# POSTECH-CVLab/InstaOrder

Measured on AMD Instinct MI355X. Metric: instance-pairs/sec (fwd+bwd), higher is better.
Workload: dtype f32; 1 GPU; InstaOrderNet_o, pair-batch 256 per GPU at 256x256x5, fp32, fwd+bwd+SGD (BASELINE.json configs[1]); inputs=resident in HBM, pairs_per_gpu=256, input_size=256, parallelism=dp1, hip_graph=True, setup_steps=0, inputs_distinct=True

## Files before the change

### include/instaorder_hip.h

```cpp
#ifndef INSTAORDER_HIP_H
#define INSTAORDER_HIP_H

#include <stddef.h>
#include <stdint.h>

#ifdef __cplusplus
extern "C" {
#endif

#define IO_OK 0
#define IO_ERR_SHAPE (-1)
#define IO_ERR_WORKSPACE (-2)
#define IO_ERR_LAUNCH (-3)
#define IO_ERR_STATE (-4)
#define IO_ERR_NODEVICE (-5)

#if !defined(__HIP__) && !defined(HIP_INCLUDE_HIP_HIP_RUNTIME_API_H)
typedef void* hipStream_t;
#endif

int io_abi_version(void);
const char* io_last_error_string(void);
int io_device_count(void);
int io_set_winograd(int on);
// ... 182 lines not shown
int io_depth_errors_median(const float* pred, const uint16_t* gt, int B, int H, int W, float gt_div, float min_depth,
                           float max_depth, double* out, float* medians, void* workspace, size_t workspace_bytes,
                           hipStream_t stream);
int io_disp_sample_points(const float* disp, int B, int H, int W, const int* points, float* values, int* decisions,
                          hipStream_t stream);
#define IO_MASK_NONZERO 0
#define IO_MASK_EQ1 1
#define IO_MASK_MAX_N 65535
int io_mask_pack(const uint8_t* masks, int n, int H, int W, int predicate, int dilate, uint32_t* bits, int64_t* stats,
                 hipStream_t stream);
int io_mask_pair_counts(const uint32_t* p_bits, int n_p, const uint32_t* q_bits, int n_q, int H, int W, int32_t* counts,
                        hipStream_t stream);
#define IO_DEPTH_SELECT_MEAN 0
#define IO_DEPTH_SELECT_MEDIAN 1
size_t io_instance_depth_select_workspace_bytes(int n, int H, int W);
int io_instance_depth_select(const float* disp, int H, int W, const uint8_t* masks, int n, int method, float* value, float* lo,
                             float* hi, int32_t* k, void* workspace, size_t workspace_bytes, hipStream_t stream);
int io_conv2d_fwd_bnstats_dt(const void* x, const void* w, void* y, int N, int H, int W, int Cin, int Cout, int R, int S,
                             int stride, int pad, int G, const float* gamma, const float* beta, float* running_mean,
                             float* running_var, float momentum, float eps, float* mean, float* rstd, float* scale,
                             float* shift, float* workspace, size_t workspace_floats, int dtype, int gw,
                             hipStream_t stream);
int io_conv2d_dgrad_bnbwd_dt(const void* dy, const void* wt, void* dz, int N, int H, int W, int Cin, int Cout, int R, int S,
                             int pad, const void* y, int G, const float* gamma, const float* mean, const float* rstd,
                             const float* scale, const float* shift, float* dgamma, float* dbeta, void* dyb,
                             float* workspace, size_t workspace_floats, int dtype, int gw, hipStream_t stream);
size_t io_stem_packed_floats(int real_channels);
size_t io_stem_wgrad_exact_workspace_bytes(int N, int H, int W, int real_channels);
int io_stem_fwd_bnstats_exact(const float* x8, const float* w, float* y, int N, int H, int W, int real_channels, int G,
                              const float* gamma, const float* beta, float* running_mean, float* running_var,
                              float momentum, float eps, float* mean, float* rstd, float* scale, float* shift,
                              float* workspace, size_t workspace_floats, float* packed, hipStream_t stream);
int io_stem_wgrad_exact(const float* x8, const float* dy, float* dw, int N, int H, int W, int real_channels,
                        void* workspace, size_t workspace_bytes, float* packed, hipStream_t stream);
int io_stem_wgrad_exact_bn(const float* x8, const float* da, const float* y, float* dw, int N, int H, int W,
                           int real_channels, int G, const float* gamma, const float* mean, const float* rstd,
                           const float* scale, const float* shift, float* dgamma, float* dbeta, float* coef,
                           float* bn_partial, size_t bn_partial_floats, void* workspace, size_t workspace_bytes,
                           float* packed, hipStream_t stream);

size_t io_bn_tile_partial_floats(int M, int C, int G);
int io_bn_bwd_coefs_dt(const void* dz, const void* y, int M, int C, int G, const float* gamma, const float* mean,
                       const float* rstd, float* dgamma, float* dbeta, float* coef, float* partial,
                       size_t partial_floats, int dtype, hipStream_t stream);
int io_bn_bwd_coefs_from_tile_partials(float* p1, float* p2, int M, int C, int G, const float* gamma, const float* mean,
                                       const float* rstd, float* dgamma, float* dbeta, float* coef, hipStream_t stream);
typedef struct io_dgrad_fused {
    const void* xb_y;
    const float* xb_coef;
    void* xb_dy_out;
    const void* add;
    const void* relu_mask;
    const void* ep_y;
    const float *ep_mean, *ep_rstd, *ep_scale, *ep_shift;
    void* ep_act_out;
    float *ep_p1, *ep_p2;
    float* wino_scratch;
    size_t wino_scratch_floats;
    const uint32_t* relu_maskbits;
} io_dgrad_fused;
int io_conv2d_dgrad_fused_dt(const void* dy, const void* wt, void* dx, int N, int H, int W, int Cin, int Cout, int R,
                             int S, int pad, int G, const io_dgrad_fused* f, int dtype, hipStream_t stream);
size_t io_conv2d_wino_scratch_floats(int Cin, int Cout);
int io_conv2d_fwd_wino(const float* x, const float* w, float* y, int N, int H, int W, int Cin, int Cout, int G,
                       const float* in_mean, const float* in_scale, const float* in_shift, const float* gamma,
                       const float* beta, float* running_mean, float* running_var, float momentum, float eps, float* mean,
                       float* rstd, float* scale, float* shift, float* workspace, size_t workspace_floats,
                       float* wino_scratch, size_t wino_floats, hipStream_t stream);
int io_conv2d_fwd_xf_dt(const void* x, const void* w, void* y, int N, int H, int W, int Cin, int Cout, int R, int S,
                        int stride, int pad, int G, const float* in_mean, const float* in_scale, const float* in_shift,
                        const float* gamma, const float* beta, float* running_mean, float* running_var, float momentum, float eps,
                        float* mean, float* rstd, float* scale, float* shift, float* workspace, size_t workspace_floats,
                        int dtype, hipStream_t stream);
int io_conv2d_fwd_resid(const float* y3, const float* identity, const float* w, float* y, float* out, int N, int H, int W,
                        int Cin, int Cout, int G, const float* in_mean, const float* in_scale, const float* in_shift,
                        const float* gamma, const float* beta, float* running_mean, float* running_var, float momentum,
                        float eps, float* mean, float* rstd, float* scale, float* shift, float* workspace,
                        size_t workspace_floats, hipStream_t stream);
int io_conv2d_fwd_resid_dt(const void* y3, const void* second, const void* w, void* y, void* out, uint32_t* out_bits, int N,
                           int H, int W, int Cin, int Cout, int G, int two, const float* ta, const float* tb, const float* tc,
                           float* tile_mean, float* tile_m2, int dtype, hipStream_t stream);
int io_set_bf16_p256_xop(int on);
int io_get_bf16_p256_xop(void);
typedef struct io_weight_desc {
    long src, dst_op, dst_t, dst_g;
    int Co, Ci, T, Cop, Cip;
} io_weight_desc;
int io_weights_prepare(const void* table, int n, const float* params, void* ops, int dtype, hipStream_t stream);
int io_weights_unpack_grads(const void* table, int n, const float* gk, float* grads, hipStream_t stream);
size_t io_stem_wgrad_bf16_workspace_bytes(void);
int io_stem_wgrad_bn_bf16(const void* x8, const void* da, const void* y, float* dw, int N, int H, int W, int G,
                          const float* gamma, const float* mean, const float* rstd, const float* scale, const float* shift,
                          float* dgamma, float* dbeta, float* coef, float* bn_partial, size_t bn_partial_floats,
                          void* workspace, size_t workspace_bytes, hipStream_t stream);
int io_debug_last_wgrad_route(void);
int io_maxpool_fwd_xf_dt(const void* x, int N, int H, int W, int C, void* out, uint32_t* idx, int G,
                         const float* in_mean, const float* in_scale, const float* in_shift, int dtype,
                         hipStream_t stream);
int io_conv2d_fwd_bias_dt(const void* x, const void* w, void* y, int N, int H, int W, int Cin, int Cout, int R, int S,
                          int stride, int pad, const float* bias, const void* add, int relu, int dtype, int gw,
                          hipStream_t stream);
int io_maxpool_fwd_dt(const void* x, int N, int H, int W, int C, void* out, uint32_t* idx, int dtype, hipStream_t stream);
int io_maxpool_bwd_dt(const void* dy, const uint32_t* idx, int N, int H, int W, int C, void* dx, int dtype,
                      hipStream_t stream);
int io_avgpool_fc_fwd_dt(const void* x, int N, int HW, int C, const float* w0, const float* b0, int K0, const float* w1,
                         const float* b1, int K1, float* pooled, float* logits, int dtype, hipStream_t stream);
int io_avgpool_fc_bwd_dt(const float* dlogits, const float* pooled, int N, int HW, int C, const float* w0, int K0,
                         const float* w1, int K1, const void* relu_mask, void* dx, float* dw0, float* db0, float* dw1,
                         float* db1, int dtype, hipStream_t stream);

typedef struct io_pair_desc {
    int64_t image_off;
    int64_t mask1_off, mask2_off;
    int32_t H, W;
    int32_t x, y, w, h;
    int32_t flip;
    int32_t interp;
} io_pair_desc;
int io_pair_planes_u8(const uint8_t* arena, size_t arena_bytes, const io_pair_desc* desc_dev,
                      const io_pair_desc* desc_host, int P, int S, const double* mean3, const double* std3, float* rgb,
                      float* modal1, float* modal2, hipStream_t stream);
int io_pair_planes_u8_hw(const uint8_t* arena, size_t arena_bytes, const io_pair_desc* desc_dev,
                         const io_pair_desc* desc_host, int P, int SH, int SW, const double* mean3, const double* std3,
                         float* rgb, float* modal1, float* modal2, hipStream_t stream);

#define IO_RLE_LDS_RUNS 4096
typedef struct io_rle_desc {
    int64_t ends_off;
    int32_t n_runs;
    int32_t H, W;
    int32_t value;
    int64_t out_off;
} io_rle_desc;
int io_rle_decode_u8(const uint32_t* ends_dev, size_t ends_count, const io_rle_desc* desc_dev,
                     const io_rle_desc* desc_host, int n, uint8_t* out, size_t out_bytes, hipStream_t stream);
int io_rle_lds_runs(void);

typedef struct io_prof_entry {
    char name[48];
    long launches;
    double total_ms;
    double flops;
    double bytes;
    double flops_executed;
} io_prof_entry;
int io_prof_begin(void);
int io_prof_begin_ex(int share_events);
int io_prof_end(io_prof_entry* out, int max_entries);
int io_prof_launches(io_prof_entry* out, int max_entries);

#ifdef __cplusplus
}
#endif
#endif
```

### instaorder_amd/_lib.py

```python
import ctypes as C
import os

_HERE = os.path.dirname(os.path.abspath(__file__))
LIB_PATH = os.environ.get("IO_LIB_PATH") or os.path.join(_HERE, "libinstaorder_hip.so")
_lib = None

c_float_p = C.c_void_p


def csrc_digest():
    import glob
    import hashlib
    h = hashlib.sha256()
    files = sorted(glob.glob(os.path.join(_HERE, "csrc", "*.hip")) + glob.glob(os.path.join(_HERE, "csrc", "*.h")))
    files.append(os.path.join(os.path.dirname(_HERE), "include", "instaorder_hip.h"))
    for f in files:
        h.update(os.path.basename(f).encode())
        h.update(open(f, "rb").read())
    return h.hexdigest()[:16]


class TensorInfo(C.Structure):
    _fields_ = [("name", C.c_char * 64), ("kind", C.c_int), ("ndim", C.c_int), ("shape", C.c_long * 4),
                ("offset", C.c_long), ("numel_storage", C.c_long), ("cin_storage", C.c_int),
                ("bn_index", C.c_int), ("running_offset", C.c_long)]


class PairDesc(C.Structure):
    _fields_ = [("image_off", C.c_int64), ("mask1_off", C.c_int64), ("mask2_off", C.c_int64), ("H", C.c_int32),
                ("W", C.c_int32), ("x", C.c_int32), ("y", C.c_int32), ("w", C.c_int32), ("h", C.c_int32),
                ("flip", C.c_int32), ("interp", C.c_int32)]


class RleDesc(C.Structure):
    _fields_ = [("ends_off", C.c_int64), ("n_runs", C.c_int32), ("H", C.c_int32), ("W", C.c_int32),
                ("value", C.c_int32), ("out_off", C.c_int64)]


class DgradFused(C.Structure):
    _fields_ = [(n, C.c_void_p) for n in ("xb_y", "xb_coef", "xb_dy_out", "add", "relu_mask", "ep_y", "ep_mean", "ep_rstd",
                                          "ep_scale", "ep_shift", "ep_act_out", "ep_p1", "ep_p2", "wino_scratch")] + \
               [("wino_scratch_floats", C.c_size_t), ("relu_maskbits", C.c_void_p)]


class ProfEntry(C.Structure):
    _fields_ = [("name", C.c_char * 48), ("launches", C.c_long), ("total_ms", C.c_double),
                ("flops", C.c_double), ("bytes", C.c_double), ("flops_executed", C.c_double)]


class ClipState(C.Structure):
    _fields_ = [("norm", C.c_float), ("coef", C.c_float), ("nonfinite", C.c_int), ("reserved0", C.c_int),
                ("steps", C.c_uint64), ("clipped", C.c_uint64), ("skipped", C.c_uint64), ("reserved", C.c_uint64 * 3)]


_P, _I, _L, _F, _Z = C.c_void_p, C.c_int, C.c_long, C.c_float, C.c_size_t
_D = C.c_double

SIGNATURES = {
    "io_abi_version": (_I, []),
    "io_last_error_string": (C.c_char_p, []),
    "io_device_count": (_I, []),
    "io_set_winograd": (_I, [_I]),
    "io_get_winograd": (_I, []),
    "io_set_bf16_p256": (_I, [_I]),
    "io_get_bf16_p256": (_I, []),
    "io_set_bf16_p256_xop": (_I, [_I]),
    "io_get_bf16_p256_xop": (_I, []),
    "io_conv2d_fwd_resid_dt": (_I, [_P, _P, _P, _P, _P, _P, _I, _I, _I, _I, _I, _I, _I, _P, _P, _P, _P, _P, _I, _P]),
    "io_debug_last_nt_route": (_I, []),
    "io_conv2d_fwd": (_I, [_P, _P, _P, _I, _I, _I, _I, _I, _I, _I, _I, _I, _P]),
    "io_conv2d_bnstats_workspace_floats": (_Z, [_I, _I, _I, _I, _I, _I, _I, _I, _I]),
    "io_conv2d_fwd_bnstats": (_I, [_P, _P, _P, _I, _I, _I, _I, _I, _I, _I, _I, _I, _I, _P, _P, _P, _P, _F, _F, _P, _P,
                                   _P, _P, _P, _Z, _P]),
    "io_conv2d_dgrad": (_I, [_P, _P, _P, _P, _P, _I, _I, _I, _I, _I, _I, _I, _I, _I, _P]),
    "io_conv2d_dgrad_bnbwd": (_I, [_P, _P, _P, _I, _I, _I, _I, _I, _I, _I, _I, _P, _I, _P, _P, _P, _P, _P, _P, _P, _P,
                                   _P, _Z, _P]),
    "io_conv2d_wgrad_workspace_bytes": (_Z, [_I, _I, _I, _I, _I, _I, _I, _I, _I]),
    "io_conv2d_wgrad": (_I, [_P, _P, _P, _I, _I, _I, _I, _I, _I, _I, _I, _I, _P, _Z, _P]),
    "io_filter_transpose": (_I, [_P, _I, _I, _I, _P, _P]),
    "io_bn_partial_floats": (_Z, [_I, _I, _I]),
    "io_bn_stats_finalize": (_I, [_P, _I, _I, _I, _P, _P, _P, _P, _F, _F, _P, _P, _P, _P, _P, _Z, _P]),
    "io_bn_eval_prepare": (_I, [_I, _P, _P, _P, _P, _F, _P, _P, _P, _P]),
    "io_bn_apply": (_I, [_P, _I, _I, _I, _I, _P, _P, _P, _P, _P, _P, _P, _I, _P, _P]),
    "io_bn_bwd": (_I, [_P, _P, _P, _P, _P, _I, _I, _I, _P, _P, _P, _P, _P, _P, _P, _P, _Z, _P, _P]),
    "io_maxpool_fwd": (_I, [_P, _I, _I, _I, _I, _P, _P, _P]),
    "io_maxpool_bwd": (_I, [_P, _P, _I, _I, _I, _I, _P, _P]),
    "io_avgpool_fc_fwd": (_I, [_P, _I, _I, _I, _P, _P, _I, _P, _P, _I, _P, _P, _P]),
    "io_avgpool_fc_bwd": (_I, [_P, _P, _I, _I, _I, _P, _I, _P, _I, _P, _P, _P, _P, _P, _P, _P]),
    "io_pack_planes_nhwc8": (_I, [C.POINTER(C.c_void_p), C.POINTER(C.c_long), _I, _I, _I, _I, _P, _P]),
    "io_pair_planes_u8": (_I, [_P, _Z, _P, _P, _I, _I, _P, _P, _P, _P, _P, _P]),
    "io_pair_planes_u8_hw": (_I, [_P, _Z, _P, _P, _I, _I, _I, _P, _P, _P, _P, _P, _P]),
    "io_rle_decode_u8": (_I, [_P, _Z, _P, _P, _I, _P, _Z, _P]),
    "io_rle_lds_runs": (_I, []),
    "io_order_loss": (_I, [_P, _I, _I, _I, _I, _P, _P, _P, _F, _F, _F, _P, _P, _P]),
    "io_sgd_momentum": (_I, [_P, _P, _P, _Z, _F, _F, _F, _P]),
    "io_adam_step": (_I, [_P, _P, _P, _P, _Z, _D, _D, _D, _F, _F, _D, _D, _P]),
    "io_grad_norm": (_I, [_P, _Z, C.POINTER(C.c_size_t), _I, _F, _P, _Z, _P, _P, _P]),
    "io_grad_norm_workspace_bytes": (_Z, [_Z, _I]),
    "io_grad_norm_chunk_floats": (_I, []),
    "io_sgd_momentum_clipped": (_I, [_P, _P, _P, _Z, _F, _F, _F, _P, _P]),
    "io_adam_step_clipped": (_I, [_P, _P, _P, _P, _Z, _D, _D, _D, _F, _F, _D, _D, _P, _P]),
    "io_net_create": (_P, [_I, _I, C.POINTER(C.c_int)]),
    "io_net_destroy": (None, [_P]),
    "io_net_param_floats": (_L, [_P]),
    "io_net_running_floats": (_L, [_P]),
    "io_net_num_tensors": (_I, [_P]),
    "io_net_tensor_info": (_I, [_P, _I, C.POINTER(TensorInfo)]),
    "io_net_num_logits": (_I, [_P]),
    "io_net_workspace_bytes": (_Z, [_P, _I, _I, _I]),
    "io_net_workspace_bytes_hw": (_Z, [_P, _I, _I, _I]),
    "io_net_forward_eval_hw": (_I, [_P, _P, _P, _P, _I, _I, _I, _P, _Z, _P, _P]),
    "io_net_activation_offset": (_L, [_P, _I, _I, _I]),
    "io_net_forward": (_I, [_P, _P, _P, _P, _I, _I, _I, _I, _P, _Z, _P, _P]),
    "io_net_backward": (_I, [_P, _P, _P, _P, _P, _I, _I, _I, _P, _Z, _P]),
    "io_net_backward_num_stages": (_I, [_P]),
    "io_net_backward_stages": (_I, [_P, _P, _P, _P, _P, _I, _I, _I, _P, _Z, _I, _I, _P]),
    "io_net_set_dtype": (_I, [_P, _I]),
    "io_net_get_dtype": (_I, [_P]),
    "io_pack_planes_nhwc8_dt": (_I, [_P, _P, _I, _I, _I, _I, _P, _I, _P]),
    "io_conv2d_fwd_dt": (_I, [_P, _P, _P, _I, _I, _I, _I, _I, _I, _I, _I, _I, _I, _I, _P]),
    "io_conv2d_dgrad_dt": (_I, [_P, _P, _P, _P, _P, _I, _I, _I, _I, _I, _I, _I, _I, _I, _I, _P]),
    "io_conv2d_wgrad_dt": (_I, [_P, _P, _P, _I, _I, _I, _I, _I, _I, _I, _I, _I, _P, _Z, _I, _I, _P]),
    "io_filter_prepare": (_I, [_P, _I, _I, _I, _P, _I, _I, _P]),
    "io_bn_stats_finalize_dt": (_I, [_P, _I, _I, _I, _P, _P, _P, _P, _F, _F, _P, _P, _P, _P, _P, _Z, _I, _P]),
    "io_bn_apply_dt": (_I, [_P, _I, _I, _I, _I, _P, _P, _P, _P, _P, _P, _P, _I, _P, _I, _P]),
    "io_bn_apply_bits_dt": (_I, [_P, _I, _I, _I, _I, _P, _P, _P, _P, _P, _P, _P, _P, _P, _I, _P]),
    "io_bn_bwd_dt": (_I, [_P, _P, _P, _P, _P, _I, _I, _I, _P, _P, _P, _P, _P, _P, _P, _P, _Z, _P, _I, _P]),
    "io_gconv_pack": (_I, [_P, _I, _I, _I, _P, _P, _I, _P]),
    "io_gconv_unpack_grad": (_I, [_P, _I, _I, _I, _P, _P]),
    "io_gconv2d_fwd": (_I, [_P, _P, _P, _I, _I, _I, _I, _I, _I, _I, _I, _I, _P]),
    "io_gconv2d_dgrad": (_I, [_P, _P, _P, _I, _I, _I, _I, _I, _I, _I, _I, _I, _P]),
    "io_gconv2d_wgrad_workspace_bytes": (_Z, [_I, _I, _I, _I, _I, _I, _I, _I]),
    "io_gconv2d_wgrad": (_I, [_P, _P, _P, _I, _I, _I, _I, _I, _I, _I, _I, _P, _Z, _I, _P]),
    "io_upsample2x_bilinear_fwd": (_I, [_P, _I, _I, _I, _I, _I, _P, _I, _P]),
    "io_upsample2x_bilinear_bwd": (_I, [_P, _I, _I, _I, _I, _I, _P, _I, _P]),
    "io_bias_act": (_I, [_P, _P, _I, _I, _I, _P, _I, _P]),
    "io_relu_bwd": (_I, [_P, _P, _Z, _P, _I, _P]),
    "io_add": (_I, [_P, _P, _Z, _P, _I, _P]),
    "io_colsum_partial_floats": (_Z, [_I, _I]),
    "io_colsum": (_I, [_P, _I, _I, _P, _P, _Z, _I, _P]),
    "io_head1_fwd": (_I, [_P, _I, _I, _I, _P, _P, _I, _P, _I, _P]),
    "io_head1_bwd": (_I, [_P, _P, _P, _I, _I, _I, _P, _I, _P, _P, _P, _P, _Z, _I, _P]),
    "io_conv2d_fwd_bnstats_dt": (_I, [_P, _P, _P, _I, _I, _I, _I, _I, _I, _I, _I, _I, _I, _P, _P, _P, _P, _F, _F, _P,
                                      _P, _P, _P, _P, _Z, _I, _I, _P]),
    "io_conv2d_fwd_bias_dt": (_I, [_P, _P, _P, _I, _I, _I, _I, _I, _I, _I, _I, _I, _P, _P, _I, _I, _I, _P]),
    "io_stem_packed_floats": (_Z, [_I]),
    "io_stem_wgrad_exact_workspace_bytes": (_Z, [_I, _I, _I, _I]),
    "io_stem_fwd_bnstats_exact": (_I, [_P, _P, _P, _I, _I, _I, _I, _I, _P, _P, _P, _P, _F, _F, _P, _P, _P, _P, _P, _Z, _P,
                                       _P]),
# ... 80 lines not shown
```

### instaorder_amd/csrc/capi.hip

```cpp
#include <stdarg.h>
#include <stdio.h>
#include <stdlib.h>
#include <string.h>

#include "io_common.h"

static thread_local char g_err[512] = "";

void io_set_error(const char* fmt, ...) {
    va_list ap;
    va_start(ap, fmt);
    vsnprintf(g_err, sizeof(g_err), fmt, ap);
    va_end(ap);
}

int io_check_launch(const char* what) {
    hipError_t e = hipGetLastError();
    if (e != hipSuccess) {
        io_set_error("%s: %s", what, hipGetErrorString(e));
        return IO_ERR_LAUNCH;
    }
    return IO_OK;
}

extern "C" int io_abi_version(void) { return 1; }

static std::atomic<int> g_wino{-1};
bool io_wino_on() {
    int v = g_wino.load(std::memory_order_relaxed);
    if (v < 0) {
        const char* e = getenv("IO_WINOGRAD");
        v = (e && e[0] == '0') ? 0 : 1;
        g_wino.store(v, std::memory_order_relaxed);
    }
    return v != 0;
}
extern "C" int io_get_winograd(void) { return io_wino_on() ? 1 : 0; }
extern "C" int io_set_winograd(int on) {
    const int prev = io_wino_on() ? 1 : 0;
    g_wino.store(on ? 1 : 0, std::memory_order_relaxed);
    return prev;
}
extern "C" const char* io_last_error_string(void) { return g_err; }

extern "C" int io_device_count(void) {
    int n = 0;
    if (hipGetDeviceCount(&n) != hipSuccess) {
        (void)hipGetLastError();
        return 0;
    }
    int ok = 0;
    for (int i = 0; i < n; ++i) {
        hipDeviceProp_t p;
        if (hipGetDeviceProperties(&p, i) == hipSuccess && strncmp(p.gcnArchName, "gfx950", 6) == 0) ++ok;
    }
    return ok;
}

IoConvGeom io_geom_fwd(int N, int H, int W, int Cin, int Cout, int R, int S, int stride, int pad) {
    IoConvGeom g;
    memset(&g, 0, sizeof(g));
    g.N = N; g.Hi = H; g.Wi = W; g.Ci = Cin;
    g.Ho = (H + 2 * pad - R) / stride + 1;
    g.Wo = (W + 2 * pad - S) / stride + 1;
    g.Co = Cout;
    g.outH = g.Ho; g.outW = g.Wo;
    g.os = 1; g.ooh = 0; g.oow = 0;
    g.is = stride;
    g.Th = R; g.Tw = S;
    g.dh0 = -pad; g.dhs = 1; g.dw0 = -pad; g.dws = 1;
    g.r0 = 0; g.rs = 1; g.s0 = 0; g.ss = 1;
    g.S = S; g.wT = R * S;
    io_geom_finish(g);
    return g;
}

IoConvGeom io_geom_dgrad(int N, int H, int W, int Cin, int Cout, int R, int S, int stride, int pad, int ph,
                         int pw) {
    IoConvGeom g;
    memset(&g, 0, sizeof(g));
    const int Hy = (H + 2 * pad - R) / stride + 1, Wy = (W + 2 * pad - S) / stride + 1;
    g.N = N; g.Hi = Hy; g.Wi = Wy; g.Ci = Cout;
    g.Ho = (H - ph + stride - 1) / stride;
    g.Wo = (W - pw + stride - 1) / stride;
    g.Co = Cin;
    g.outH = H; g.outW = W;
    g.os = stride; g.ooh = ph; g.oow = pw;
    g.is = 1;
    const int rf = (ph + pad) % stride, sf = (pw + pad) % stride;
    g.Th = rf < R ? (R - rf + stride - 1) / stride : 0;
    g.Tw = sf < S ? (S - sf + stride - 1) / stride : 0;
    g.dh0 = (ph + pad - rf) / stride; g.dhs = -1;
    g.dw0 = (pw + pad - sf) / stride; g.dws = -1;
    g.r0 = rf; g.rs = stride; g.s0 = sf; g.ss = stride;
    g.S = S; g.wT = R * S;
    io_geom_finish(g);
    return g;
}

int io_run_dgrad(const void* dy, const void* wt, void* dx, const void* add, const void* mask, int N, int H,
                 int W, int Cin, int Cout, int R, int S, int stride, int pad, hipStream_t st, const IoBwStats* bw,
                 int dt, int gw) {
    IO_REQUIRE(!bw || !bw->y || stride == 1, IO_ERR_SHAPE, "dgrad: fused BN-backward reductions need a stride-1 convolution");
    IO_REQUIRE(!bw || !bw->xb_a || stride == 1 || (R == 1 && S == 1 && pad == 0), IO_ERR_SHAPE,
               "dgrad: the operand transform needs a stride-1 convolution or a strided 1x1 one");
    for (int ph = 0; ph < stride; ++ph)
        for (int pw = 0; pw < stride; ++pw) {
            IoConvGeom g = io_geom_dgrad(N, H, W, Cin, Cout, R, S, stride, pad, ph, pw);
            g.gw = gw;
            if (g.Ho <= 0 || g.Wo <= 0) continue;
            if ((g.Th == 0 || g.Tw == 0) && add == dx && !mask) continue;
            int rc = io_launch_conv_nt(g, dy, wt, dx, add, mask, 0, st, nullptr, nullptr, bw, dt, dt);
            if (rc) return rc;
        }
    return IO_OK;
}

extern "C" int io_conv2d_fwd(const float* x, const float* w, float* y, int N, int H, int W, int Cin, int Cout,
                             int R, int S, int stride, int pad, hipStream_t st) {
    IoConvGeom g = io_geom_fwd(N, H, W, Cin, Cout, R, S, stride, pad);
    return io_launch_conv_nt(g, x, w, y, nullptr, nullptr, Cin == 8, st);
}

// ... 587 lines not shown
```

### instaorder_amd/csrc/conv_igemm.hip

```cpp
#include <string.h>
#include <stdlib.h>

#include "io_common.h"

namespace {

constexpr int kThreads = 256;

__device__ __forceinline__ f32x4 ld4(const float* p) { return *reinterpret_cast<const f32x4*>(p); }
template <typename T> __device__ __forceinline__ void pin(T& v) { asm volatile("" : "+v"(v)); }
__device__ __forceinline__ void st4(float* p, f32x4 v) { *reinterpret_cast<f32x4*>(p) = v; }

__device__ __forceinline__ int xcd_remap(int b, int nwg) {
    const int q = nwg >> 3, r = nwg & 7, x = b & 7, i = b >> 3;
    return (x < r ? x * (q + 1) : r * (q + 1) + (x - r) * q) + i;
}

__device__ __forceinline__ int sdiv(int n, float rd) { return (int)(((float)n + 0.5f) * rd); }
__device__ __forceinline__ int stem_kp(int wT, int cr) { return (wT * cr + 31) / 32 * 32; }
__device__ __forceinline__ int fdiv(int n, IoFastDiv f) {
    return f.shift < 0 ? n : (int)(__umulhi((unsigned)n, f.magic) >> f.shift);
}

typedef unsigned u32x4 __attribute__((ext_vector_type(4)));
constexpr unsigned kInvalidOff = 0xFFFFFFFFu;
constexpr int kStAux = 2;
constexpr int kTrBkm = 64;
constexpr int kTrMinB = 2;
constexpr int kTrStages = 2;
__device__ __forceinline__ __amdgpu_buffer_rsrc_t make_rsrc(const void* p, unsigned bytes) {
    return __builtin_amdgcn_make_buffer_rsrc(const_cast<void*>(p), 0, bytes, 0x00020000);
}
__device__ __forceinline__ __amdgpu_buffer_rsrc_t make_rsrc_at(const void* p, size_t base, size_t total) {
    const size_t rest = total > base ? total - base : 0;
    return make_rsrc(static_cast<const char*>(p) + base, rest > 0xFFFFFFFFull ? 0xFFFFFFFFu : (unsigned)rest);
}
__device__ __forceinline__ f32x4 bld4(__amdgpu_buffer_rsrc_t r, unsigned off) {
    return __builtin_bit_cast(f32x4, __builtin_amdgcn_raw_buffer_load_b128(r, off, 0, 0));
}
template <typename T> __device__ __forceinline__ f32x4 bldv(__amdgpu_buffer_rsrc_t r, unsigned off);
template <> __device__ __forceinline__ f32x4 bldv<float>(__amdgpu_buffer_rsrc_t r, unsigned off) { return bld4(r, off); }
template <> __device__ __forceinline__ f32x4 bldv<bf16_t>(__amdgpu_buffer_rsrc_t r, unsigned off) {
    typedef unsigned u32x2 __attribute__((ext_vector_type(2)));
    const u32x2 q = __builtin_amdgcn_raw_buffer_load_b64(r, off, 0, 0);
    f32x4 v;
    v[0] = __builtin_bit_cast(float, q[0] << 16);
    v[1] = __builtin_bit_cast(float, q[0] & 0xffff0000u);
    v[2] = __builtin_bit_cast(float, q[1] << 16);
    v[3] = __builtin_bit_cast(float, q[1] & 0xffff0000u);
    return v;
}
template <typename T> __device__ __forceinline__ float ld_el(__amdgpu_buffer_rsrc_t r, unsigned off);
template <> __device__ __forceinline__ float ld_el<float>(__amdgpu_buffer_rsrc_t r, unsigned off) {
    return __builtin_bit_cast(float, __builtin_amdgcn_raw_buffer_load_b32(r, off, 0, 0));
}
template <> __device__ __forceinline__ float ld_el<bf16_t>(__amdgpu_buffer_rsrc_t r, unsigned off) {
    return io_bf2f(__builtin_amdgcn_raw_buffer_load_b16(r, off, 0, 0));
}
template <typename T> __device__ __forceinline__ void st_el(float v, __amdgpu_buffer_rsrc_t r, unsigned off);
template <> __device__ __forceinline__ void st_el<float>(float v, __amdgpu_buffer_rsrc_t r, unsigned off) {
    __builtin_amdgcn_raw_buffer_store_b32(__float_as_uint(v), r, off, 0, kStAux);
}
template <> __device__ __forceinline__ void st_el<bf16_t>(float v, __amdgpu_buffer_rsrc_t r, unsigned off) {
    __builtin_amdgcn_raw_buffer_store_b16(io_f2bf(v), r, off, 0, kStAux);
}
template <typename T> __device__ __forceinline__ float ld_el_s(__amdgpu_buffer_rsrc_t r, unsigned off, unsigned soff);
template <> __device__ __forceinline__ float ld_el_s<float>(__amdgpu_buffer_rsrc_t r, unsigned off, unsigned soff) {
    return __builtin_bit_cast(float, __builtin_amdgcn_raw_buffer_load_b32(r, off, soff, 0));
}
template <> __device__ __forceinline__ float ld_el_s<bf16_t>(__amdgpu_buffer_rsrc_t r, unsigned off, unsigned soff) {
    return io_bf2f(__builtin_amdgcn_raw_buffer_load_b16(r, off, soff, 0));
}
template <typename T> __device__ __forceinline__ void st_el_s(float v, __amdgpu_buffer_rsrc_t r, unsigned off, unsigned soff);
template <> __device__ __forceinline__ void st_el_s<float>(float v, __amdgpu_buffer_rsrc_t r, unsigned off, unsigned soff) {
    __builtin_amdgcn_raw_buffer_store_b32(__float_as_uint(v), r, off, soff, kStAux);
}
template <> __device__ __forceinline__ void st_el_s<bf16_t>(float v, __amdgpu_buffer_rsrc_t r, unsigned off, unsigned soff) {
    __builtin_amdgcn_raw_buffer_store_b16(io_f2bf(v), r, off, soff, kStAux);
}
typedef __bf16 bf16x8 __attribute__((ext_vector_type(8)));

template <typename TA, typename TO, int BN, int STEM, int NW, int NBUF = 2, int MINB = 1, bool BWE = false,
          bool XF = false, bool LIN = false, int XB = 0, bool WINO = false>
__global__ __launch_bounds__(NW * 64, MINB) void conv_nt_kernel(IoConvGeom g, const TA* __restrict__ in,
                                                         const TA* __restrict__ wgt, TO* __restrict__ out,
                                                         const TO* __restrict__ add,
                                                         const TO* __restrict__ mask, int ntn, size_t in_bytes,
                                                         unsigned w_bytes, size_t out_bytes,
                                                         float* __restrict__ st_mean, float* __restrict__ st_m2,
                                                         IoBwStats bw) {
    constexpr int ES = sizeof(TA), OS = sizeof(TO);
    constexpr int VE = 16 / ES;
    constexpr bool SWZ = BN == 64;
    constexpr int BM = 128, BK = 128 / ES, LDT = SWZ ? 32 : 32 + 4, NT = NW * 64;
    constexpr int CPT = ES / 2;
    constexpr int TPT = 8 / CPT;
    constexpr bool XK = STEM == 2;
    static_assert(!XK || ES == 4, "the exact-K stem is an fp32 path");
    constexpr int WN = NW / 2;
    static_assert(!WINO || (ES == 4 && OS == 4 && BN == 64 && NW == 4 && STEM == 0 && NBUF == 1 && !LIN && XB == 0),
                  "WINO: fp32, 64-wide tiles, single LDS buffer, plain / XF / BWE forms");
    constexpr int TI = WINO ? 4 : 2, TJ = BN / (32 * WN);
    constexpr int ETI = 2;
    constexpr int AROWS = WINO ? 2 * BM : BM, BROWS = WINO ? 4 * BN : BN;
    constexpr int AR = (BM * 8) / NT;
    constexpr int BR = (BN * 8) / NT;
    constexpr int RS = NT / 8;
    static_assert(TJ >= 1 && BR >= 1, "tile too small for this wave count");
    static_assert(NBUF * (BM + BN) * LDT >= NW * 32 * (BN / WN + 4), "operand LDS too small for the row epilogue");
    extern __shared__ __attribute__((aligned(16))) float smem[];
    float* sA = smem;
    float* sB = smem + NBUF * AROWS * LDT;

    const int tid = threadIdx.x, lane = tid & 63, wave = tid >> 6;
    const int wm = wave / WN, wn = wave % WN;
    const int tile = xcd_remap(blockIdx.x, gridDim.x);
    const int mt = tile / ntn;
    const int m0 = mt * BM, n0 = (tile - mt * ntn) * BN;
    const int HoWo = g.Ho * g.Wo;
    const int M = g.N * HoWo;
    const int lr = tid >> 3, kq = tid & 7;
    const int kw = g.gw ? g.gw : g.Ci;
    const int cbase = g.gw ? n0 : 0;
    const int nkc = STEM ? 1 : kw / BK;
    const int kp = XK ? stem_kp(g.wT, g.cr) : 0;
    const int nk = XK ? kp / 32 : STEM ? (g.wT + TPT - 1) / TPT : (WINO ? g.Th : g.Th * g.Tw) * nkc;

    static_assert(!LIN || STEM == 0, "LIN: regular 1x1 convolutions");
    const int n_lo = LIN ? 0 : fdiv(m0, g.fd_howo);
    const __amdgpu_buffer_rsrc_t rs_in =
        make_rsrc_at(in, LIN ? (size_t)m0 * (size_t)(g.Ci * ES) : (size_t)n_lo * (size_t)(g.Hi * g.Wi) * (size_t)(g.Ci * ES),
                     in_bytes);
    const __amdgpu_buffer_rsrc_t rs_w = make_rsrc(wgt, w_bytes);
    unsigned rowv[AR];
    int hi0[AR], wi0[AR];
    bool rvalid[AR];
#pragma unroll
    for (int j = 0; j < AR; ++j) {
        if constexpr (LIN) {
            rvalid[j] = true;
            hi0[j] = wi0[j] = 0;
            rowv[j] = (unsigned)((lr + RS * j) * g.Ci + kq * VE) * (unsigned)ES;
        } else {
            const int m = m0 + lr + RS * j;
            rvalid[j] = m < M;
            const int mm = rvalid[j] ? m : 0;
            const int n = fdiv(mm, g.fd_howo), rem = mm - n * HoWo;
            const int ho = fdiv(rem, g.fd_wo), wo = rem - ho * g.Wo;
            hi0[j] = ho * g.is;
            wi0[j] = wo * g.is;
            rowv[j] = (unsigned)((((n - n_lo) * g.Hi + hi0[j]) * g.Wi + wi0[j]) * g.Ci + (STEM ? 0 : kq * VE)) * (unsigned)ES;
        }
    }
    constexpr int AI = 2, WBR = 8;
    unsigned wrow[AI];
    int whi[AI];
    bool wl[AI], wr[AI];
    unsigned wvb[WBR];
    f32x4 wa[WINO ? AI : 1][4], wb[WINO ? WBR : 1];
    if constexpr (WINO) {
#pragma unroll
        for (int j = 0; j < AI; ++j) {
            const int m = m0 + 2 * (lr + 32 * j);
            const int n = fdiv(m, g.fd_howo), rem = m - n * HoWo;
            const int ho = fdiv(rem, g.fd_wo), wo = rem - ho * g.Wo;
            whi[j] = ho;
            wl[j] = wo > 0;
            wr[j] = wo + 2 < g.Wi;
            wrow[j] = (unsigned)((((n - n_lo) * g.Hi + ho) * g.Wi + wo) * g.Ci + kq * 4) * 4u;
        }
#pragma unroll
        for (int j = 0; j < WBR; ++j)
            wvb[j] = (unsigned)(((j >> 1) * g.Co + n0 + lr + 32 * (j & 1)) * g.Ci + kq * 4) * 4u;
    }
    unsigned wv[BR];
#pragma unroll
    for (int j = 0; j < BR; ++j)
        wv[j] = XK ? (unsigned)((n0 + lr + RS * j) * kp + kq * VE) * (unsigned)ES
                   : (unsigned)((n0 + lr + RS * j) * g.wT * kw + (STEM ? 0 : kq * VE)) * (unsigned)ES;
    const bool nopad = g.Th == 1 && g.Tw == 1 && g.dh0 == 0 && g.dw0 == 0 && g.is == 1 && g.Hi >= g.Ho &&
                       g.Wi >= g.Wo;

    f32x4 ra[AR], rb[BR];
    static_assert(!XF || STEM == 0, "input transform: regular convolutions");
    static_assert(!XB || (STEM == 0 && !XF), "backward operand transform: regular data gradients, not combined with XF");
    static_assert(XB < 2 || !BWE, "the residual forms are forward paths");
    constexpr bool XT = XF || XB;
    constexpr int XC = ES == 4 ? 1 : 2;
    f32x4 xm[XC], xs[XC], xh[XC];
    f32x4 ry[XB ? AR : 1];
    unsigned xok = 0, xaoff = 0;
    bool xside = false;
    const int xgrp = XF ? m0 / bw.in_Mg : XB ? m0 / bw.xb_Mg : 0;
    const float* const xt_s = XF ? bw.in_scale : bw.xb_a;
    const float* const xt_h = XF ? bw.in_shift : bw.xb_c;
    const float* const xt_m = XF ? bw.in_mean : bw.xb_b;
    const __amdgpu_buffer_rsrc_t rs_xs = make_rsrc(XT ? (const void*)(xt_s + (size_t)xgrp * g.Ci) : (const void*)wgt,
                                                   XT ? (unsigned)g.Ci * 4u : 0u);
    const __amdgpu_buffer_rsrc_t rs_xh = make_rsrc(XT ? (const void*)(xt_h + (size_t)xgrp * g.Ci) : (const void*)wgt,
                                                   XT ? (unsigned)g.Ci * 4u : 0u);
    const __amdgpu_buffer_rsrc_t rs_xm = make_rsrc((XT && xt_m) ? (const void*)(xt_m + (size_t)xgrp * g.Ci)
                                                                : (const void*)wgt,
                                                   (XT && xt_m) ? (unsigned)g.Ci * 4u : 0u);
    const size_t xb_base = LIN ? (size_t)m0 * (size_t)(g.Ci * ES) : (size_t)n_lo * (size_t)(g.Hi * g.Wi) * (size_t)(g.Ci * ES);
    const __amdgpu_buffer_rsrc_t rs_y = make_rsrc_at(XB ? bw.xb_y : (const void*)in, xb_base, XB ? in_bytes : xb_base);
    const __amdgpu_buffer_rsrc_t rs_side =
        make_rsrc_at((XB && bw.xb_out) ? bw.xb_out : (void*)out, xb_base, (XB && bw.xb_out && n0 == 0) ? in_bytes : xb_base);
    int th = 0, tw = 0, cc = 0;
    const float rcr = 1.0f / (float)(XK ? g.cr : 1), rS = 1.0f / (float)g.S;
    auto load_tile = [&](int kt) {
        if constexpr (XK) {
            unsigned eoff[4];
            int edh[4], edw[4];
            bool eok[4];
#pragma unroll
            for (int i = 0; i < 4; ++i) {
                const int e = kt * 32 + kq * 4 + i;
                const int tp = sdiv(e, rcr), ch = e - tp * g.cr;
                eok[i] = tp < g.wT;
                const int r = sdiv(tp, rS), s = tp - r * g.S;
                edh[i] = g.dh0 + g.dhs * r;
                edw[i] = g.dw0 + g.dws * s;
                eoff[i] = (unsigned)((edh[i] * g.Wi + edw[i]) * g.Ci + ch) * 4u;
            }
#pragma unroll
            for (int j = 0; j < AR; ++j)
#pragma unroll
                for (int i = 0; i < 4; ++i) {
                    const int hi = hi0[j] + edh[i], wi = wi0[j] + edw[i];
                    const bool ok = eok[i] && rvalid[j] && (unsigned)hi < (unsigned)g.Hi && (unsigned)wi < (unsigned)g.Wi;
                    ra[j][i] = ld_el<float>(rs_in, ok ? rowv[j] + eoff[i] : kInvalidOff);
                }
#pragma unroll
            for (int j = 0; j < BR; ++j) rb[j] = bld4(rs_w, wv[j] + (unsigned)kt * 128u);
            return;
        }
        if constexpr (LIN) {
            const unsigned koff = (unsigned)(cc * BK) * (unsigned)ES;
            if constexpr (XB) {
                xaoff = koff;
#pragma unroll
                for (int j = 0; j < AR; ++j)
                    ry[j] = __builtin_bit_cast(f32x4, __builtin_amdgcn_raw_buffer_load_b128(rs_y, rowv[j], koff, 0));
            }
            if constexpr (XT) {
                const unsigned coff = (unsigned)(cc * BK + kq * VE) * 4u;
#pragma unroll
                for (int q = 0; q < XC; ++q) {
                    xm[q] = bld4(rs_xm, coff + 16u * q);
                    xs[q] = bld4(rs_xs, coff + 16u * q);
                    xh[q] = bld4(rs_xh, coff + 16u * q);
                }
                xok = ~0u;
            }
#pragma unroll
            for (int j = 0; j < AR; ++j)
                ra[j] = __builtin_bit_cast(f32x4, __builtin_amdgcn_raw_buffer_load_b128(rs_in, rowv[j], koff, 0));
#pragma unroll
            for (int j = 0; j < BR; ++j)
                rb[j] = __builtin_bit_cast(f32x4, __builtin_amdgcn_raw_buffer_load_b128(rs_w, wv[j], koff, 0));
            return;
        }
        if constexpr (WINO) {
            const int dh = g.dh0 + g.dhs * th;
            const unsigned aoff = (unsigned)(((dh * g.Wi - 1) * g.Ci + cc * BK) * 4);
            const unsigned woff = (unsigned)((th * 4 * g.Co * g.Ci + cc * BK) * 4);
            if constexpr (XF) {
                const unsigned coff = (unsigned)(cc * BK + kq * VE) * 4u;
                xm[0] = bld4(rs_xm, coff);
                xs[0] = bld4(rs_xs, coff);
                xh[0] = bld4(rs_xh, coff);
            }
            xok = 0;
#pragma unroll
            for (int j = 0; j < AI; ++j) {
                const bool rowok = (unsigned)(whi[j] + dh) < (unsigned)g.Hi;
#pragma unroll
                for (int i = 0; i < 4; ++i) {
                    const bool ok = rowok & (i == 0 ? wl[j] : i == 3 ? wr[j] : true);
                    xok |= ok ? (1u << (j * 4 + i)) : 0u;
                    wa[j][i] = bld4(rs_in, ok ? wrow[j] + aoff + (unsigned)(i * g.Ci * 4) : kInvalidOff);
                }
            }
#pragma unroll
            for (int j = 0; j < WBR; ++j) wb[j] = bld4(rs_w, wvb[j] + woff);
            return;
        }
        int dh, dw;
        unsigned aoff, woff;
        bool tapok = true;
// ... 72 lines not shown
                    }
                }
                const f32x4 d0 = wa[j][0], d1 = wa[j][1], d2 = wa[j][2], d3 = wa[j][3];
                wa[j][0] = d0 - d2;
                wa[j][1] = d1 + d2;
                wa[j][2] = d2 - d1;
                wa[j][3] = d1 - d3;
            }
            return;
        }
        if constexpr (XF) {
#pragma unroll
            for (int j = 0; j < AR; ++j) {
                const bool ok = (xok >> j) & 1u;
                if constexpr (ES == 4) {
#pragma unroll
                    for (int e = 0; e < 4; ++e) {
                        const float v = fmaxf(__builtin_fmaf(ra[j][e] - xm[0][e], xs[0][e], xh[0][e]), 0.f);
                        ra[j][e] = ok ? v : 0.f;
                    }
                } else {
                    const u32x4 raw = __builtin_bit_cast(u32x4, ra[j]);
                    u32x4 o;
#pragma unroll
                    for (int d = 0; d < 4; ++d) {
                        const int q = d >> 1, e0 = (d & 1) * 2;
                        const float lo = __builtin_bit_cast(float, raw[d] << 16);
                        const float hi = __builtin_bit_cast(float, raw[d] & 0xffff0000u);
                        const float vl = fmaxf(__builtin_fmaf(lo - xm[q][e0], xs[q][e0], xh[q][e0]), 0.f);
                        const float vh = fmaxf(__builtin_fmaf(hi - xm[q][e0 + 1], xs[q][e0 + 1], xh[q][e0 + 1]), 0.f);
                        o[d] = ok ? io_f2bf2(vl, vh) : 0u;
                    }
                    ra[j] = __builtin_bit_cast(f32x4, o);
                }
            }
        }
        if constexpr (XB != 0) {
#pragma unroll
            for (int j = 0; j < AR; ++j) {
                const bool ok = (xok >> j) & 1u;
                if constexpr (XB == 2 && ES == 4) {
#pragma unroll
                    for (int e = 0; e < 4; ++e) {
                        const float v = __builtin_fmaf(ra[j][e] - xm[0][e], xs[0][e], xh[0][e]) + ry[j][e];
                        ra[j][e] = (ok && v > 0.f) ? v : 0.f;
                    }
                } else if constexpr (ES == 4) {
#pragma unroll
                    for (int e = 0; e < 4; ++e) {
                        const float v = __builtin_fmaf(ra[j][e], xs[0][e], __builtin_fmaf(ry[j][e], xm[0][e], xh[0][e]));
                        ra[j][e] = (ok && (XB != 3 || v > 0.f)) ? v : 0.f;
                    }
                } else {
                    const u32x4 raw = __builtin_bit_cast(u32x4, ra[j]), rwy = __builtin_bit_cast(u32x4, ry[j]);
                    u32x4 o;
#pragma unroll
                    for (int d = 0; d < 4; ++d) {
                        const int q = d >> 1, e0 = (d & 1) * 2;
                        const float lo = __builtin_bit_cast(float, raw[d] << 16);
                        const float hi = __builtin_bit_cast(float, raw[d] & 0xffff0000u);
                        const float yl = __builtin_bit_cast(float, rwy[d] << 16);
                        const float yh = __builtin_bit_cast(float, rwy[d] & 0xffff0000u);
                        float vl, vh;
                        if constexpr (XB == 2) {
                            vl = __builtin_fmaf(lo - xm[q][e0], xs[q][e0], xh[q][e0]) + yl;
                            vh = __builtin_fmaf(hi - xm[q][e0 + 1], xs[q][e0 + 1], xh[q][e0 + 1]) + yh;
                        } else {
                            vl = __builtin_fmaf(lo, xs[q][e0], __builtin_fmaf(yl, xm[q][e0], xh[q][e0]));
                            vh = __builtin_fmaf(hi, xs[q][e0 + 1], __builtin_fmaf(yh, xm[q][e0 + 1], xh[q][e0 + 1]));
                        }
                        if constexpr (XB >= 2) {
                            vl = vl > 0.f ? vl : 0.f;
                            vh = vh > 0.f ? vh : 0.f;
                        }
                        o[d] = ok ? io_f2bf2(vl, vh) : 0u;
                    }
                    ra[j] = __builtin_bit_cast(f32x4, o);
                }
            }
            if constexpr (LIN) {
#pragma unroll
                for (int j = 0; j < AR; ++j)
                    __builtin_amdgcn_raw_buffer_store_b128(__builtin_bit_cast(u32x4, ra[j]), rs_side, rowv[j], xaoff, 0);
            } else {
#pragma unroll
                for (int j = 0; j < AR; ++j)
                    __builtin_amdgcn_raw_buffer_store_b128(__builtin_bit_cast(u32x4, ra[j]), rs_side,
                                                           (xside && ((xok >> j) & 1u)) ? rowv[j] + xaoff : kInvalidOff, 0, 0);
            }
        }
    };
    auto store_tile = [&](int buf, bool xdone = false) {
        if constexpr (WINO) {
            if (!xdone) xform_tile();
            float* a = sA + lr * LDT + wchunk * 4;
            float* b = sB + lr * LDT + wchunk * 4;
#pragma unroll
            for (int j = 0; j < AI; ++j)
#pragma unroll
                for (int f = 0; f < 4; ++f) st4(a + (f * 64 + 32 * j) * LDT, wa[j][f]);
#pragma unroll
            for (int j = 0; j < WBR; ++j) st4(b + 32 * j * LDT, wb[j]);
            return;
        }
        float* a = sA + buf * BM * LDT + lr * LDT + wchunk * 4;
        float* b = sB + buf * BN * LDT + lr * LDT + wchunk * 4;
        if constexpr (XT) {
            if (!xdone) xform_tile();
        }
#pragma unroll
        for (int j = 0; j < AR; ++j) st4(a + RS * j * LDT, ra[j]);
#pragma unroll
        for (int j = 0; j < BR; ++j) st4(b + RS * j * LDT, rb[j]);
    };

    f32x16 acc[TI][TJ];
#pragma unroll
    for (int i = 0; i < TI; ++i)
#pragma unroll
        for (int j = 0; j < TJ; ++j)
#pragma unroll
            for (int r = 0; r < 16; ++r) acc[i][j][r] = 0.f;

    const int rsw = SWZ ? (lane >> 1) & 7 : 0;
    const int a_off = (wm * (WINO ? 32 : 64) + (lane & 31)) * LDT + (SWZ ? 0 : (lane >> 5) * 4);
    const int b_off = (wn * (BN / WN) + (lane & 31)) * LDT + (SWZ ? 0 : (lane >> 5) * 4);
    constexpr int FB = WINO ? 4 : TJ;
    auto read_frags = [&](int buf, int kk, f32x4 (&a)[TI], f32x4 (&b)[FB]) {
        const int koff = SWZ ? ((((lane >> 5) + kk * 2) ^ rsw) * 4) : kk * 8;
        if constexpr (WINO) {
#pragma unroll
            for (int f = 0; f < 4; ++f) {
                a[f] = ld4(sA + a_off + koff + f * 64 * LDT);
                b[f] = ld4(sB + b_off + koff + f * 64 * LDT);
            }
            return;
        }
        const float* al = sA + buf * BM * LDT + a_off + koff;
        const float* bl = sB + buf * BN * LDT + b_off + koff;
#pragma unroll
        for (int i = 0; i < TI; ++i) a[i] = ld4(al + i * 32 * LDT);
#pragma unroll
        for (int j = 0; j < TJ; ++j) b[j] = ld4(bl + j * 32 * LDT);
    };
    auto mma16 = [&](const f32x4 (&a)[TI], const f32x4 (&b)[FB]) {
        if constexpr (WINO) {
#pragma unroll
            for (int tt = 0; tt < 4; ++tt)
#pragma unroll
                for (int f = 0; f < 4; ++f)
                    acc[f][0] = __builtin_amdgcn_mfma_f32_32x32x2f32(a[f][tt], b[f][tt], acc[f][0], 0, 0, 0);
        } else if constexpr (ES == 4) {
#pragma unroll
            for (int tt = 0; tt < 4; ++tt)
#pragma unroll
                for (int i = 0; i < TI; ++i)
#pragma unroll
                    for (int j = 0; j < TJ; ++j)
                        acc[i][j] = __builtin_amdgcn_mfma_f32_32x32x2f32(a[i][tt], b[j][tt], acc[i][j], 0, 0, 0);
        } else {
#pragma unroll
            for (int i = 0; i < TI; ++i)
#pragma unroll
                for (int j = 0; j < TJ; ++j)
                    acc[i][j] = __builtin_amdgcn_mfma_f32_32x32x16_bf16(__builtin_bit_cast(bf16x8, a[i]),
                                                                        __builtin_bit_cast(bf16x8, b[j]), acc[i][j],
// ... 38 lines not shown
        for (int j = 0; j < FB; ++j) pin(fb[j]);
        if (NBUF == 1) __syncthreads();
        store_tile(nbuf, PIPE);
        __syncthreads();
        f32x4 na[TI], nb[FB];
        read_frags(nbuf, 0, na, nb);
        __builtin_amdgcn_sched_barrier(0);
        mma16(fa, fb);
#pragma unroll
        for (int i = 0; i < TI; ++i) fa[i] = na[i];
#pragma unroll
        for (int j = 0; j < FB; ++j) fb[j] = nb[j];
    }
    if (nk > 0) {
        const int buf = NBUF == 2 ? (nk - 1) & 1 : 0;
#pragma unroll
        for (int kk = 0; kk < 3; ++kk) {
            f32x4 na[TI], nb[FB];
            read_frags(buf, kk + 1, na, nb);
            mma16(fa, fb);
#pragma unroll
            for (int i = 0; i < TI; ++i) fa[i] = na[i];
#pragma unroll
            for (int j = 0; j < FB; ++j) fb[j] = nb[j];
        }
        mma16(fa, fb);
    }

    if constexpr (WINO) {
#pragma unroll
        for (int r = 0; r < 16; ++r) {
            const float m1 = acc[1][0][r], m2 = acc[2][0][r];
            acc[0][0][r] = acc[0][0][r] + m1 + m2;
            acc[1][0][r] = m1 - m2 - acc[3][0][r];
        }
    }
    constexpr int RQ = WINO ? 2 : 1, RI = WINO ? 1 : 32;
    if (st_mean) {
        __syncthreads();
        float* red = smem;
        const int nvalid = min(BM, M - m0);
        float cmean[TJ];
#pragma unroll
        for (int pass = 0; pass < 2; ++pass) {
#pragma unroll
            for (int j = 0; j < TJ; ++j) {
                float sacc = 0.f;
#pragma unroll
                for (int i = 0; i < ETI; ++i)
#pragma unroll
                    for (int r = 0; r < 16; ++r) {
                        const int m = m0 + wm * 64 + RI * i + RQ * ((r & 3) + 8 * (r >> 2) + 4 * (lane >> 5));
                        const float v = acc[i][j][r];
                        const float d = pass == 0 ? v : (v - cmean[j]) * (v - cmean[j]);
                        sacc += m < M ? d : 0.f;
                    }
                sacc += __shfl_xor(sacc, 32, 64);
                if (lane < 32) red[wm * BN + wn * (BN / WN) + j * 32 + lane] = sacc;
            }
            __syncthreads();
#pragma unroll
            for (int j = 0; j < TJ; ++j) {
                const int cl = wn * (BN / WN) + j * 32 + (lane & 31);
                const float tot = red[cl] + red[BN + cl];
                if (pass == 0) {
                    cmean[j] = tot / (float)nvalid;
                } else if (wm == 0 && lane < 32) {
                    const size_t o = (size_t)mt * g.Co + n0 + cl;
                    st_mean[o] = cmean[j];
                    st_m2[o] = tot;
                }
            }
            __syncthreads();
        }
    }

    const bool dense = (g.os == 1) && (g.Ho == g.outH) && (g.Wo == g.outW);
    const int opix_lo = LIN ? m0 : n_lo * g.outH * g.outW;
    const size_t out_base = (size_t)opix_lo * (size_t)(g.Co * OS);
    const __amdgpu_buffer_rsrc_t rs_out = make_rsrc_at(out, out_base, out_bytes);
    const __amdgpu_buffer_rsrc_t rs_add = make_rsrc_at(add ? (const void*)add : (const void*)out, out_base, out_bytes);
    const __amdgpu_buffer_rsrc_t rs_mask = make_rsrc_at(mask ? (const void*)mask : (const void*)out, out_base, out_bytes);
    const __amdgpu_buffer_rsrc_t rs_bwy = make_rsrc_at(bw.y ? bw.y : (const void*)out, out_base, out_bytes);
    float bw_mu[TJ], bw_rs[TJ], bw_sc[TJ], bw_sh[TJ], bw_s1[TJ], bw_s2[TJ];
    if constexpr (BWE) {
        const int gcol = (m0 / bw.Mg) * g.Co + n0 + wn * (BN / WN) + (lane & 31);
#pragma unroll
        for (int j = 0; j < TJ; ++j) {
            bw_mu[j] = bw.mean[gcol + j * 32];
            bw_rs[j] = bw.rstd[gcol + j * 32];
            bw_sc[j] = bw.mscale ? bw.mscale[gcol + j * 32] : 0.f;
            bw_sh[j] = bw.mscale ? bw.mshift[gcol + j * 32] : 0.f;
            bw_s1[j] = 0.f;
            bw_s2[j] = 0.f;
        }
        const unsigned colb2 = (unsigned)(n0 + wn * (BN / WN) + (lane & 31)) * (unsigned)OS;
        const unsigned rowstep = (unsigned)g.Co * (unsigned)OS;
        const unsigned lane_base = (unsigned)(m0 - opix_lo + wm * 64 + RQ * 4 * (lane >> 5)) * rowstep + colb2;
        const __amdgpu_buffer_rsrc_t rs_add0 = add ? rs_add : make_rsrc(out, 0);
        const __amdgpu_buffer_rsrc_t rs_mask0 = mask ? rs_mask : make_rsrc(out, 0);
        const bool nomask = mask == nullptr;
        const __amdgpu_buffer_rsrc_t rs_aout = make_rsrc_at(bw.a_out ? bw.a_out : (void*)out, out_base,
                                                            bw.a_out ? out_bytes : out_base);
        constexpr bool ROWS = OS == 2 && BN == 128;
        constexpr int WC = BN / WN, EPP = WC + 4, LPR = WC / 4, RPI = 64 / LPR, NI = 32 / RPI;
        float* ep = smem + wave * (32 * EPP);
        if (ROWS) __syncthreads();
#pragma unroll
        for (int i = 0; i < ETI; ++i) {
#pragma unroll
            for (int j = 0; j < TJ; ++j) {
                const unsigned voff = lane_base + (unsigned)(i * RI) * rowstep + (unsigned)j * 32u * OS;
                float av[16], mv[16], yv[16];
#pragma unroll
                for (int r = 0; r < 16; ++r) yv[r] = ld_el_s<TO>(rs_bwy, voff, (unsigned)(RQ * ((r & 3) + 8 * (r >> 2))) * rowstep);
#pragma unroll
                for (int r = 0; r < 16; ++r) av[r] = ld_el_s<TO>(rs_add0, voff, (unsigned)(RQ * ((r & 3) + 8 * (r >> 2))) * rowstep);
#pragma unroll
                for (int r = 0; r < 16; ++r) mv[r] = ld_el_s<TO>(rs_mask0, voff, (unsigned)(RQ * ((r & 3) + 8 * (r >> 2))) * rowstep);
#pragma unroll
                for (int r = 0; r < 16; ++r) {
                    float v = acc[i][j][r] + av[r];
                    v = (mv[r] > 0.f || nomask) ? v : 0.f;
                    const float t = __builtin_fmaf(yv[r] - bw_mu[j], bw_sc[j], bw_sh[j]);
                    if (bw.mscale) v = t > 0.f ? v : 0.f;
                    bw_s1[j] += v;
                    bw_s2[j] += v * ((yv[r] - bw_mu[j]) * bw_rs[j]);
                    if constexpr (ROWS) ep[((r & 3) + 8 * (r >> 2) + 4 * (lane >> 5)) * EPP + j * 32 + (lane & 31)] = v;
                    else st_el_s<TO>(v, rs_out, voff, (unsigned)(RQ * ((r & 3) + 8 * (r >> 2))) * rowstep);
                    st_el_s<TO>(fmaxf(t, 0.f), rs_aout, voff, (unsigned)(RQ * ((r & 3) + 8 * (r >> 2))) * rowstep);
                }
            }
            if constexpr (ROWS) {
#pragma unroll
                for (int k = 0; k < NI; ++k) {
                    const int row = k * RPI + lane / LPR, cc = (lane % LPR) * 4;
                    const f32x4 q = ld4(ep + row * EPP + cc);
                    typedef unsigned u32x2_ __attribute__((ext_vector_type(2)));
                    const u32x2_ pk = {io_f2bf2(q[0], q[1]), io_f2bf2(q[2], q[3])};
                    __builtin_amdgcn_raw_buffer_store_b64(
                        pk, rs_out, (unsigned)((m0 - opix_lo + wm * 64 + i * 32 + row) * g.Co + n0 + wn * WC + cc) * 2u, 0,
                        kStAux);
                }
            }
        }
    }
    if constexpr (!BWE) {
    float ep_bias[TJ];
#pragma unroll
    for (int j = 0; j < TJ; ++j) ep_bias[j] = bw.bias ? bw.bias[n0 + wn * (BN / WN) + j * 32 + (lane & 31)] : 0.f;
    if constexpr (LIN) {
        const unsigned rowstep = (unsigned)g.Co * (unsigned)OS;
        const unsigned lane_base = (unsigned)((wm * 64 + 4 * (lane >> 5)) * g.Co + n0 + wn * (BN / WN) + (lane & 31)) * (unsigned)OS;
        if constexpr (OS == 2 && BN == 128) {
            if (!add && !mask) {
                constexpr int WC = BN / WN, EPP = WC + 4, LPR = WC / 4, RPI = 64 / LPR, NI = 32 / RPI;
                __syncthreads();
                float* ep = smem + wave * (32 * EPP);
#pragma unroll
                for (int i = 0; i < ETI; ++i) {
#pragma unroll
                    for (int j = 0; j < TJ; ++j)
#pragma unroll
                        for (int r = 0; r < 16; ++r) {
                            float v = acc[i][j][r];
                            if (bw.bias) {
                                v += ep_bias[j];
                                v = (bw.relu && v < 0.f) ? 0.f : v;
                            }
                            ep[((r & 3) + 8 * (r >> 2) + 4 * (lane >> 5)) * EPP + j * 32 + (lane & 31)] = v;
                        }
#pragma unroll
                    for (int k = 0; k < NI; ++k) {
                        const int row = k * RPI + lane / LPR, cc = (lane % LPR) * 4;
                        const f32x4 q = ld4(ep + row * EPP + cc);
                        typedef unsigned u32x2_ __attribute__((ext_vector_type(2)));
                        const u32x2_ pk = {io_f2bf2(q[0], q[1]), io_f2bf2(q[2], q[3])};
                        __builtin_amdgcn_raw_buffer_store_b64(
                            pk, rs_out, (unsigned)((wm * 64 + i * 32 + row) * g.Co + n0 + wn * WC + cc) * 2u, 0, kStAux);
                    }
                }
                return;
            }
        }
#pragma unroll
        for (int i = 0; i < ETI; ++i) {
#pragma unroll
            for (int j = 0; j < TJ; ++j) {
                const unsigned voff = lane_base + (unsigned)(i * 32) * rowstep + (unsigned)j * 32u * OS;
                if (add) {
                    float av[16];
#pragma unroll
                    for (int r = 0; r < 16; ++r) av[r] = ld_el_s<TO>(rs_add, voff, (unsigned)((r & 3) + 8 * (r >> 2)) * rowstep);
#pragma unroll
                    for (int r = 0; r < 16; ++r) acc[i][j][r] += av[r];
                }
                if (bw.bias) {
#pragma unroll
                    for (int r = 0; r < 16; ++r) {
                        const float v = acc[i][j][r] + ep_bias[j];
                        acc[i][j][r] = (bw.relu && v < 0.f) ? 0.f : v;
                    }
                }
                if (mask) {
                    float mv[16];
#pragma unroll
                    for (int r = 0; r < 16; ++r) mv[r] = ld_el_s<TO>(rs_mask, voff, (unsigned)((r & 3) + 8 * (r >> 2)) * rowstep);
#pragma unroll
                    for (int r = 0; r < 16; ++r) acc[i][j][r] = mv[r] > 0.f ? acc[i][j][r] : 0.f;
                }
#pragma unroll
                for (int r = 0; r < 16; ++r) {
                    const float v = acc[i][j][r];
                    st_el_s<TO>(v, rs_out, voff, (unsigned)((r & 3) + 8 * (r >> 2)) * rowstep);
                }
            }
        }
    } else {
    const unsigned colb = (unsigned)(n0 + wn * (BN / WN) + (lane & 31)) * (unsigned)OS;
    constexpr unsigned JS = 32u * OS;
#pragma unroll
    for (int i = 0; i < ETI; ++i) {
        unsigned rowb[16];
#pragma unroll
        for (int r = 0; r < 16; ++r) {
            const int m = m0 + wm * 64 + RI * i + RQ * ((r & 3) + 8 * (r >> 2) + 4 * (lane >> 5));
            const bool ok = m < M;
            int pix = ok ? m : m0;
            if (!dense) {
                const int n = fdiv(pix, g.fd_howo), rem = pix - n * HoWo;
                const int ho = fdiv(rem, g.fd_wo), wo = rem - ho * g.Wo;
                pix = (n * g.outH + (ho * g.os + g.ooh)) * g.outW + (wo * g.os + g.oow);
            }
            rowb[r] = ok ? (unsigned)((pix - opix_lo) * g.Co) * (unsigned)OS + colb : kInvalidOff;
        }
        if (add) {
#pragma unroll
            for (int j = 0; j < TJ; ++j) {
                float av[16];
#pragma unroll
                for (int r = 0; r < 16; ++r)
                    av[r] = ld_el<TO>(rs_add, rowb[r] == kInvalidOff ? kInvalidOff : rowb[r] + j * JS);
#pragma unroll
                for (int r = 0; r < 16; ++r) acc[i][j][r] += av[r];
            }
        }
        if (bw.bias) {
#pragma unroll
            for (int j = 0; j < TJ; ++j)
#pragma unroll
                for (int r = 0; r < 16; ++r) {
                    const float v = acc[i][j][r] + ep_bias[j];
                    acc[i][j][r] = (bw.relu && v < 0.f) ? 0.f : v;
                }
        }
        if (mask) {
#pragma unroll
            for (int j = 0; j < TJ; ++j) {
                float mv[16];
#pragma unroll
                for (int r = 0; r < 16; ++r)
                    mv[r] = ld_el<TO>(rs_mask, rowb[r] == kInvalidOff ? kInvalidOff : rowb[r] + j * JS);
#pragma unroll
                for (int r = 0; r < 16; ++r) acc[i][j][r] = mv[r] > 0.f ? acc[i][j][r] : 0.f;
            }
        }
#pragma unroll
        for (int r = 0; r < 16; ++r) {
#pragma unroll
            for (int j = 0; j < TJ; ++j) {
                const float v = acc[i][j][r];
                st_el<TO>(v, rs_out, rowb[r] == kInvalidOff ? kInvalidOff : rowb[r] + j * JS);
            }
        }
    }
    }
    }
    if constexpr (BWE) {
        __syncthreads();
        float* red = smem;
#pragma unroll
        for (int j = 0; j < TJ; ++j) {
            const float a = bw_s1[j] + __shfl_xor(bw_s1[j], 32, 64);
            const float b = bw_s2[j] + __shfl_xor(bw_s2[j], 32, 64);
            if (lane < 32) {
                const int cl = wn * (BN / WN) + j * 32 + lane;
                red[wm * BN + cl] = a;
                red[2 * BN + wm * BN + cl] = b;
            }
        }
        __syncthreads();
        if (wm == 0 && lane < 32) {
#pragma unroll
            for (int j = 0; j < TJ; ++j) {
                const int cl = wn * (BN / WN) + j * 32 + lane;
                const size_t o = (size_t)mt * g.Co + n0 + cl;
                bw.p1[o] = red[cl] + red[BN + cl];
                bw.p2[o] = red[2 * BN + cl] + red[3 * BN + cl];
            }
        }
    }
}

template <typename TX, typename TDY, int BMO, int BNC, int STEM, bool TR = false, bool W4 = false, int NBUF = 2,
          int MINB = 1>
__global__ __launch_bounds__(kThreads, MINB) void conv_wgrad_kernel(IoConvGeom g, const TX* __restrict__ in,
                                                             const TDY* __restrict__ dy,
                                                             float* __restrict__ dst, int ntile_c, int tiles,
                                                             int kps, size_t in_bytes, size_t dy_bytes) {
    constexpr int BKM = 32;
    constexpr int TI = BMO / 64, TJ = BNC / 64;
    constexpr int QA = BMO / 4, QB = BNC / 4;
    constexpr int RA = (BKM * QA) / kThreads;
    constexpr int RB = (BKM * QB) / kThreads;
    constexpr int SA = kThreads / QA, SB = kThreads / QB;
    static_assert(!TR || (STEM == 0 && sizeof(TX) == 4 && sizeof(TDY) == 4), "transposed staging: fp32, not the stem");
    constexpr int LDT = 36;
    constexpr int NA = TR ? 4 : RA, NB = TR ? 4 : RB;
    extern __shared__ __attribute__((aligned(16))) float smem[];
    float* sA = smem;
    float* sB = smem + (TR ? NBUF * BMO * LDT : NBUF * BKM * BMO);

    const int tid = threadIdx.x, lane = tid & 63, wave = tid >> 6;
    const int wm = wave >> 1, wn = wave & 1;
    const int HoWo = g.Ho * g.Wo;
    const int M = g.N * HoWo;
    const int T = g.Th * g.Tw;

    const int logical = xcd_remap(blockIdx.x, gridDim.x);
    const int split = logical / tiles, tile = logical - split * tiles;
    const int per_o = STEM ? ntile_c : T * ntile_c;
    const int ot = tile / per_o;
    const int rem0 = tile - ot * per_o;
    const int o0 = ot * BMO;
    int tap = 0, c0;
    if (STEM) {
        c0 = rem0 * BNC;
    } else {
        tap = rem0 / ntile_c;
        c0 = g.gw ? o0 : (rem0 - tap * ntile_c) * BNC;
    }
    const int qa = tid % QA, ra0 = tid / QA;
    const int qb = tid % QB, rb0 = tid / QB;
    const bool actA = !TR || ra0 < BKM / 4, actB = !TR || rb0 < BKM / 4;

    constexpr bool XK = STEM >= 2;
    static_assert(!XK || sizeof(TX) == 4, "the exact-K stem gathers fp32 dwords");
// ... 1447 lines not shown
                if (bw.bias) {
                    v += bias;
                    v = (bw.relu && v < 0.f) ? 0.f : v;
                }
                st_el_s<float>(v, rs_out, lane_off, (unsigned)(4 * ((r & 3) + 8 * (r >> 2)) + i) * rowstep);
            }
    }
}

__global__ __launch_bounds__(256) void wino4_filter_kernel(const float* __restrict__ w, float* __restrict__ U, int Co,
                                                          int Ci, int S, int r0, int rs, int s0, int ss, int dw0,
                                                          int dws) {
    const int th = blockIdx.y, c4n = Ci / 4;
    const int idx = blockIdx.x * 256 + threadIdx.x;
    if (idx >= Co * c4n) return;
    const int o = idx / c4n, c = (idx - o * c4n) * 4;
    f32x4 gq[3];
#pragma unroll
    for (int j = 0; j < 3; ++j) {
        const int tw = (j - 1 - dw0) * dws;
        const int tap = (r0 + rs * th) * S + s0 + ss * tw;
        gq[j] = ld4(w + ((size_t)o * (3 * S) + tap) * Ci + c);
    }
    const size_t plane = (size_t)Co * Ci;
    float* dst = U + (size_t)th * 6 * plane + (size_t)o * Ci + c;
    const f32x4 s02 = gq[0] + gq[2], q02 = gq[0] + 4.f * gq[2];
    st4(dst, 0.25f * gq[0]);
    st4(dst + plane, (-1.0f / 6.0f) * (s02 + gq[1]));
    st4(dst + 2 * plane, (-1.0f / 6.0f) * (s02 - gq[1]));
    st4(dst + 3 * plane, (1.0f / 24.0f) * (q02 + 2.f * gq[1]));
    st4(dst + 4 * plane, (1.0f / 24.0f) * (q02 - 2.f * gq[1]));
    st4(dst + 5 * plane, gq[2]);
}

__global__ __launch_bounds__(256) void wino_filter_kernel(const float* __restrict__ w, float* __restrict__ U, int Co,
                                                         int Ci, int S, int r0, int rs, int s0, int ss, int dw0,
                                                         int dws) {
    const int th = blockIdx.y, c4n = Ci / 4;
    const int idx = blockIdx.x * 256 + threadIdx.x;
    if (idx >= Co * c4n) return;
    const int o = idx / c4n, c = (idx - o * c4n) * 4;
    f32x4 gq[3];
#pragma unroll
    for (int j = 0; j < 3; ++j) {
        const int tw = (j - 1 - dw0) * dws;
        const int tap = (r0 + rs * th) * S + s0 + ss * tw;
        gq[j] = ld4(w + ((size_t)o * (3 * S) + tap) * Ci + c);
    }
    const size_t plane = (size_t)Co * Ci;
    float* dst = U + (size_t)th * 4 * plane + (size_t)o * Ci + c;
    st4(dst, gq[0]);
    st4(dst + plane, 0.5f * (gq[0] + gq[1] + gq[2]));
    st4(dst + 2 * plane, 0.5f * (gq[0] - gq[1] + gq[2]));
    st4(dst + 3 * plane, gq[2]);
}

__global__ __launch_bounds__(256) void splitk_reduce_kernel(const float* __restrict__ partial,
                                                           float* __restrict__ dst, size_t n4, int splits) {
    __shared__ f32x4 red[8][32];
    const int tx = threadIdx.x & 31, ty = threadIdx.x >> 5;
    const size_t i = (size_t)blockIdx.x * 32 + tx;
    const bool ok = i < n4;
    const f32x4* p4 = reinterpret_cast<const f32x4*>(partial);
    f32x4 s = {0.f, 0.f, 0.f, 0.f};
    if (ok)
        for (int z0 = ty; z0 < splits; z0 += 64) {
            f32x4 v[8];
#pragma unroll
            for (int u = 0; u < 8; ++u) {
                const int z = z0 + 8 * u;
                const f32x4 zero = {0.f, 0.f, 0.f, 0.f};
                v[u] = z < splits ? p4[(size_t)z * n4 + i] : zero;
            }
#pragma unroll
            for (int u = 0; u < 8; ++u) s += v[u];
        }
    red[ty][tx] = s;
    __syncthreads();
    if (ty == 0 && ok) {
#pragma unroll
        for (int k = 1; k < 8; ++k) s += red[k][tx];
        reinterpret_cast<f32x4*>(dst)[i] = s;
    }
}

template <typename T>
__global__ __launch_bounds__(256) void pack_sign_bits_kernel(const T* __restrict__ t, uint32_t* __restrict__ bits,
                                                             size_t nwords) {
    const size_t i = (size_t)blockIdx.x * 256 + threadIdx.x;
    if (i >= nwords) return;
    const T* p = t + i * 32;
    uint32_t w = 0;
#pragma unroll
    for (int q = 0; q < 8; ++q) {
        const f32x4 v = io_ldv(p + 4 * q);
#pragma unroll
        for (int e = 0; e < 4; ++e) w |= (v[e] > 0.f ? 1u : 0u) << (4 * q + e);
    }
    bits[i] = w;
}

inline size_t io_filter_row(const IoConvGeom& g) {
    return g.cr ? (size_t)io_stem_kp(g.wT, g.cr) : (size_t)g.wT * (g.gw ? g.gw : g.Ci);
}

struct WgradPlan {
    int bmo, bnc, ntile_c, tiles, splits, kps;
};

WgradPlan plan_wgrad(const IoConvGeom& g, int stem, bool fp32 = true) {
    WgradPlan p;
    const long M = (long)g.N * g.Ho * g.Wo;
    p.bmo = (g.Co % 128 == 0) ? 128 : 64;
    if (stem) {
        p.bnc = 64;
        p.ntile_c = g.cr ? io_stem_kp(g.wT, g.cr) / 64 + (io_stem_kp(g.wT, g.cr) % 64 != 0)
                         : io_cdiv((long)g.wT * g.Ci, 64);
        p.tiles = (g.Co / p.bmo) * p.ntile_c;
    } else if (g.gw) {
        p.bmo = p.bnc = g.gw;
        p.ntile_c = 1;
        p.tiles = (g.Co / p.bmo) * g.Th * g.Tw;
    } else {
        p.bnc = (g.Ci % 128 == 0) ? 128 : 64;
        p.ntile_c = g.Ci / p.bnc;
        p.tiles = (g.Co / p.bmo) * g.Th * g.Tw * p.ntile_c;
    }
    if (p.tiles < 1) p.tiles = 1;
    const bool fp32_tr = fp32 && !stem && !g.gw && p.bmo == 128 && p.bnc == 128;
    const int nkt = io_cdiv(M, 32);
    int want = (fp32_tr ? (p.tiles >= 128 ? 2304 : 768) : 1024) / p.tiles;
    int maxs = nkt / 8 > 0 ? nkt / 8 : 1;
    p.splits = want < maxs ? want : maxs;
    if (p.splits < 1) p.splits = 1;
    p.kps = io_cdiv(nkt, p.splits);
    p.splits = io_cdiv(nkt, p.kps);
    return p;
}

bool wgrad_wino_shape_ok(const IoConvGeom& g, int stem) {
    return !stem && !g.gw && !g.cr && g.Th == 3 && g.Tw == 3 && g.S == 3 && g.wT == 9 && g.is == 1 &&
           g.os == 1 && g.Hi == g.Ho && g.Wi == g.Wo && g.dh0 == -1 && g.dhs == 1 && g.dw0 == -1 && g.dws == 1 &&
           g.rs == 1 && g.ss == 1 && g.r0 == 0 && g.s0 == 0 && g.Wo % 8 == 0 && ((long)g.N * g.Ho * g.Wo) % 64 == 0 &&
           g.Ci % 64 == 0 && g.Co % 64 == 0;
}
bool wgrad_wino_ok(const IoConvGeom& g, int stem) { return io_wino_on() && wgrad_wino_shape_ok(g, stem); }
WgradPlan plan_wgrad_wino(const IoConvGeom& g) {
    WgradPlan p;
    p.bmo = p.bnc = 64;
    p.ntile_c = g.Ci / 64;
    p.tiles = (g.Co / 64) * 3 * p.ntile_c;
    const int nkt = (int)(((long)g.N * g.Ho * g.Wo) / 64);
    const int want = 1024 / p.tiles, maxs = nkt / 8 > 0 ? nkt / 8 : 1;
    p.splits = want < maxs ? want : maxs;
    if (p.splits < 1) p.splits = 1;
    p.kps = io_cdiv(nkt, p.splits);
    p.splits = io_cdiv(nkt, p.kps);
    return p;
}

}

size_t io_conv_wgrad_partial_bytes(const IoConvGeom& g, int stem) {
    const int s0 = plan_wgrad(g, stem, true).splits, s1 = plan_wgrad(g, stem, false).splits;
    int splits = s0 > s1 ? s0 : s1;
    if (wgrad_wino_shape_ok(g, stem)) {
        const int sw = plan_wgrad_wino(g).splits;
        if (sw > splits) splits = sw;
    }
    size_t need = splits == 1 ? 0 : (size_t)splits * g.Co * io_filter_row(g) * sizeof(float);
    if (stem && g.cr && io_stem_rows_ok(g)) {
        const size_t rows = (size_t)io_stem_wgrad_rows_max_blocks() * g.Co * io_filter_row(g) * sizeof(float);
        if (rows > need) need = rows;
    }
    if (stem && !g.cr && g.Ci == 8 && g.Co == 64 && g.Wo == 128)
        if (io_stem_wgrad_halo_partial_bytes() > need) need = io_stem_wgrad_halo_partial_bytes();
    if (!stem && io_wgrad_halo3_shape(g) && io_wgrad_halo3_partial_bytes() > need) need = io_wgrad_halo3_partial_bytes();
    return need;
}

static std::atomic<int> g_last_wgrad_route{0};
extern "C" int io_debug_last_wgrad_route(void) { return g_last_wgrad_route.load(std::memory_order_relaxed); }
static std::atomic<int> g_last_route{0};
extern "C" int io_debug_last_nt_route(void) { return g_last_route.load(std::memory_order_relaxed); }

int io_launch_conv_nt(const IoConvGeom& g, const void* in, const void* wgt, void* out, const void* add,
                      const void* mask, int stem, hipStream_t st, float* st_mean, float* st_m2,
                      const IoBwStats* bw, int dt_in, int dt_out) {
    IoBwStats bws;
    memset(&bws, 0, sizeof(bws));
    if (bw) {
        bws = *bw;
        const long Mchk = (long)g.N * g.Ho * g.Wo;
        IO_REQUIRE(!bws.y || (g.os == 1 && g.Ho == g.outH && g.Wo == g.outW && bws.Mg > 0 && bws.Mg % 128 == 0 &&
                              Mchk % 128 == 0 && Mchk % bws.Mg == 0),
                   IO_ERR_SHAPE, "conv_nt: fused BN-backward reductions need a dense output and 128 | rows per group | M");
        IO_REQUIRE(!bws.xb_res || (bws.xb_a && !bws.y && dt_in == dt_out), IO_ERR_SHAPE,
                   "conv_nt: the residual operand form is a forward path (no BatchNorm-backward epilogue)");
        IO_REQUIRE(!bws.xb_a || (bws.xb_b && bws.xb_c && bws.xb_y && !bws.in_scale && !stem && !g.gw && g.is == 1 &&
                                 g.Hi == g.Ho && g.Wi == g.Wo &&
                                 bws.xb_Mg > 0 && bws.xb_Mg % 128 == 0 && Mchk % bws.xb_Mg == 0 && g.dhs * g.dhs == 1 &&
                                 g.dws * g.dws == 1 && g.dh0 * (g.dh0 + g.dhs * (g.Th - 1)) <= 0 &&
                                 g.dw0 * (g.dw0 + g.dws * (g.Tw - 1)) <= 0),
                   IO_ERR_SHAPE,
                   "conv_nt: the backward operand transform needs a stride-1 same-size data gradient whose taps include "
                   "the centre, and 128 | rows per group | M");
    }
    IO_REQUIRE(!(stem && bws.y), IO_ERR_SHAPE, "conv_nt: the stem has no BatchNorm-backward epilogue");
    IO_REQUIRE(!bws.a_out || (bws.y && bws.mscale && bws.mshift), IO_ERR_SHAPE,
               "conv_nt: the activation side output needs the BatchNorm-backward epilogue with its mask tables");
    IO_REQUIRE(!bws.in_scale || (!stem && !bws.y && bws.in_shift && bws.in_Mg > 0 && bws.in_Mg % 128 == 0 && !g.gw),
               IO_ERR_SHAPE, "conv_nt: the input transform needs a regular forward convolution and 128 | rows per group");
    IO_REQUIRE((st_mean == nullptr) == (st_m2 == nullptr), IO_ERR_SHAPE, "conv_nt: statistics outputs come in pairs");
    IO_REQUIRE(!st_mean || (g.os == 1 && g.Ho == g.outH && g.Wo == g.outW && !add && !mask), IO_ERR_SHAPE,
               "conv_nt: fused statistics need a plain dense forward convolution");
    IO_REQUIRE(g.Co % 64 == 0, IO_ERR_SHAPE, "conv_nt: Co=%d must be a multiple of 64", g.Co);
    const int es = io_dtype_bytes(dt_in), os = io_dtype_bytes(dt_out);
    IO_REQUIRE(!g.cr || (stem && dt_in == IO_F32 && dt_out == IO_F32 && g.cr > 0 && g.cr <= 8), IO_ERR_SHAPE,
               "conv_nt: the exact-K mode is for the fp32 stem (1..8 real channels)");
    if (stem)
        IO_REQUIRE(g.Ci == 8, IO_ERR_SHAPE, "conv_nt(stem): needs the packed input with Ci=8 (5 padded)");
    else
        IO_REQUIRE(g.Ci % (128 / es) == 0, IO_ERR_SHAPE, "conv_nt: Ci=%d must be a multiple of %d", g.Ci, 128 / es);
    IO_REQUIRE(g.N > 0 && g.Ho > 0 && g.Wo > 0 && g.Hi > 0 && g.Wi > 0, IO_ERR_SHAPE,
               "conv_nt: empty tensor (N=%d, in %dx%d, out %dx%d)", g.N, g.Hi, g.Wi, g.Ho, g.Wo);
    const long M = (long)g.N * g.Ho * g.Wo;
    IO_REQUIRE(M > 0 && M < (1L << 31), IO_ERR_SHAPE, "conv_nt: bad M=%ld", M);
    const double w_b = (double)es * g.Co * (double)io_filter_row(g);
    const double span = 128.0 / ((double)g.Ho * g.Wo) + 2.0;
    IO_REQUIRE(w_b < 4.0e9 && span * es * g.Hi * g.Wi * g.Ci < 4.0e9 && span * os * g.outH * g.outW * g.Co < 4.0e9,
               IO_ERR_SHAPE, "conv_nt: filter or per-tile sample span larger than 4 GB (32-bit offsets)");
    IO_REQUIRE((double)g.N * g.Hi * g.Wi < 2.0e9 && (double)g.N * g.outH * g.outW < 2.0e9, IO_ERR_SHAPE,
               "conv_nt: more than 2^31 pixels");
    const size_t in_bytes = (size_t)es * g.N * g.Hi * g.Wi * g.Ci;
    const size_t out_bytes = (size_t)os * g.N * g.outH * g.outW * g.Co;
    const unsigned w_bytes = (unsigned)w_b;
    if (dt_in == IO_BF16 && dt_out == IO_BF16 && stem && !add && !mask) {
        const int rs = io_launch_conv_stem_halo(g, in, wgt, out, st, st_mean, st_m2, bw ? &bws : nullptr, in_bytes, w_bytes,
                                                out_bytes);
        if (rs <= 0) {
            g_last_route.store(3, std::memory_order_relaxed);
            return rs;
        }
    }
    if (dt_in == IO_BF16 && dt_out == IO_BF16 && !stem) {
        const int rh = io_launch_conv_halo3(g, in, wgt, out, add, mask, st, st_mean, st_m2, bw ? &bws : nullptr, in_bytes,
                                            w_bytes, out_bytes);
        if (rh <= 0) {
            g_last_route.store(2, std::memory_order_relaxed);
            return rh;
        }
        const int rc = io_launch_conv_p256(g, in, wgt, out, add, mask, st, st_mean, st_m2, bw ? &bws : nullptr, in_bytes,
                                           w_bytes, out_bytes);
        if (rc <= 0) {
            g_last_route.store(1, std::memory_order_relaxed);
            return rc;
        }
    }
    g_last_route.store(0, std::memory_order_relaxed);
    IO_REQUIRE(!bws.xb_bits || (bws.xb_res && bws.xb_out), IO_ERR_SHAPE,
               "conv_nt: xb_bits is the mask of the residual forms' side output (needs xb_res and xb_out)");
    static std::atomic<int> small_tiles_c{-1};
    int small_tiles = small_tiles_c.load(std::memory_order_relaxed);
    if (small_tiles < 0) {
        const char* e = getenv("IO_NT_SMALL_TILES");
        small_tiles = e ? atoi(e) : 256;
        small_tiles_c.store(small_tiles, std::memory_order_relaxed);
    }
    const long tiles128 = (long)io_cdiv(M, 128) * (g.Co / 128);
    const int bn = g.gw ? g.gw : ((g.Co % 128 == 0 && tiles128 > small_tiles) ? 128 : 64);
    IO_REQUIRE(!g.gw || (g.gw == 64 && !stem && g.Ci == g.Co), IO_ERR_SHAPE,
               "conv_nt: grouped mode needs a 64-channel window and Ci == Co");
    const int ntn = g.Co / bn;
    const long tiles = (long)io_cdiv(M, 128) * ntn;
    IO_REQUIRE(tiles < (1L << 31), IO_ERR_SHAPE, "conv_nt: grid too large");
    dim3 grid((unsigned)tiles), block(kThreads);
    const bool lin = !stem && !g.gw && g.Th * g.Tw == 1 && g.is == 1 && g.os == 1 && g.dh0 == 0 && g.dw0 == 0 &&
                     g.Hi == g.Ho && g.Wi == g.Wo && g.outH == g.Ho && g.outW == g.Wo && M % 128 == 0 &&
                     128.0 * g.Ci * es < 4.0e9 && 128.0 * g.Co * os < 4.0e9;
    IO_REQUIRE(!bws.xb_res || lin, IO_ERR_SHAPE, "conv_nt: the residual operand form needs a dense 1x1 stride-1 GEMM on whole tiles");
    if (io_wino_on() && bws.wino_u && !stem && !g.gw && dt_in == IO_F32 && dt_out == IO_F32 && g.Th == 3 && g.Tw == 3 &&
        g.S == 3 && g.wT == 9 && g.is == 1 && g.os == 1 && g.Hi == g.Ho && g.Wi == g.Wo && g.outH == g.Ho &&
        g.outW == g.Wo && g.Wo % 2 == 0 && M % 128 == 0 && g.Ci % 32 == 0 && !add && !mask && !bws.xb_a &&
        g.dhs * g.dhs == 1 && g.dws * g.dws == 1 && g.dw0 * (g.dw0 + 2 * g.dws) == -1 && g.rs == 1 && g.ss == 1 &&
        !(bws.y && bws.in_scale) && 12.0 * g.Co * g.Ci * 4.0 < 4.0e9) {
        const double kred9 = 9.0 * g.Ci;
        const bool wino4 = g.Wo % 4 == 0 && M % 256 == 0 && g.Ci % 16 == 0 && (!bws.y || bws.Mg % 256 == 0) &&
                           (!bws.in_scale || bws.in_Mg % 256 == 0) && 18.0 * g.Co * g.Ci * 4.0 < 4.0e9;
        const double fl9 = 2.0 * (double)M * g.Co * kred9;
        IoProfScope prof(IO_PROF_CONV_WINO, fl9,
                         (double)os * M * g.Co * (1.0 + (bws.y ? 1.0 : 0.0)) +
                             (double)es * ((double)g.N * g.Hi * g.Wi * g.Ci + (double)g.Co * kred9), st,
                         wino4 ? fl9 * 0.5 : fl9 * (2.0 / 3.0));
        if (wino4) {
            hipLaunchKernelGGL(wino4_filter_kernel, dim3((unsigned)io_cdiv((long)g.Co * g.Ci / 4, 256), 3), dim3(256), 0, st,
                               (const float*)wgt, bws.wino_u, g.Co, g.Ci, g.S, g.r0, g.rs, g.s0, g.ss, g.dw0, g.dws);
            const unsigned u_bytes = (unsigned)(18.0 * g.Co * g.Ci * 4.0);
            const int ntw = g.Co / 64;
            dim3 grid4((unsigned)((M / 256) * ntw));
            const long hw = (long)g.Ho * g.Wo;
            const bool halo = g.Wo <= 64 && 256 % g.Wo == 0 &&
                              (hw % 256 == 0 || (256 % hw == 0 && (256 / hw) * (g.Ho + 2) * (g.Wo / 4) <= 96));
            const size_t lds4 = (size_t)6 * ((halo ? 96 : 64) + 64) * 16 * sizeof(float);
#define IO_LAUNCH_W4_(BWE_, XF_, HALO_)                                                                                 \
    hipLaunchKernelGGL((conv_wino4_kernel<BWE_, XF_, HALO_>), grid4, block, lds4, st, g, (const float*)in,              \
                       (const float*)bws.wino_u, (float*)out, ntw, in_bytes, u_bytes, out_bytes, st_mean, st_m2, bws)
            if (halo) {
                if (bws.y) IO_LAUNCH_W4_(true, false, true);
                else if (bws.in_scale) IO_LAUNCH_W4_(false, true, true);
                else IO_LAUNCH_W4_(false, false, true);
            } else {
                if (bws.y) IO_LAUNCH_W4_(true, false, false);
                else if (bws.in_scale) IO_LAUNCH_W4_(false, true, false);
                else IO_LAUNCH_W4_(false, false, false);
            }
#undef IO_LAUNCH_W4_
            return io_check_launch("conv_nt(wino4)");
        }
        hipLaunchKernelGGL(wino_filter_kernel, dim3((unsigned)io_cdiv((long)g.Co * g.Ci / 4, 256), 3), dim3(256), 0, st,
                           (const float*)wgt, bws.wino_u, g.Co, g.Ci, g.S, g.r0, g.rs, g.s0, g.ss, g.dw0, g.dws);
        const unsigned wu_bytes = (unsigned)(12.0 * g.Co * g.Ci * 4.0);
        const int ntw = g.Co / 64;
        dim3 gridw((unsigned)((M / 128) * ntw));
        const size_t ldsz = (size_t)(256 + 256) * 32 * sizeof(float);
#define IO_LAUNCH_WINO_(BWE_, XF_)                                                                                    \
    do {                                                                                                             \
        static std::atomic<unsigned long long> attr_done{0};                                                         \
        if (io_first_on_device(attr_done))                                                                           \
            (void)hipFuncSetAttribute(                                                                               \
                (const void*)conv_nt_kernel<float, float, 64, 0, 4, 1, 2, BWE_, XF_, false, 0, true>,                \
                hipFuncAttributeMaxDynamicSharedMemorySize, (int)ldsz);                                              \
        hipLaunchKernelGGL((conv_nt_kernel<float, float, 64, 0, 4, 1, 2, BWE_, XF_, false, 0, true>), gridw, block,  \
                           ldsz, st, g, (const float*)in, (const float*)bws.wino_u, (float*)out, (const float*)nullptr, \
                           (const float*)nullptr, ntw, in_bytes, wu_bytes, out_bytes, st_mean, st_m2, bws);          \
    } while (0)
        if (bws.y) IO_LAUNCH_WINO_(true, false);
        else if (bws.in_scale) IO_LAUNCH_WINO_(false, true);
        else IO_LAUNCH_WINO_(false, false);
#undef IO_LAUNCH_WINO_
        return io_check_launch("conv_nt(wino)");
    }
    const double kred = stem ? (double)g.wT * 5.0 : (double)g.Th * g.Tw * (g.gw ? g.gw : g.Ci);
    IoProfScope prof(stem ? IO_PROF_CONV_STEM : (bn == 128 ? IO_PROF_CONV_NT128 : IO_PROF_CONV_NT64),
                     2.0 * (double)M * g.Co * kred,
                     (double)os * M * g.Co * (1.0 + (add ? 1.0 : 0.0) + (mask ? 1.0 : 0.0) + ((bw && bw->y) ? 1.0 : 0.0)) +
                         (double)es * ((kred > 0.0 ? (double)g.N * g.Hi * g.Wi * g.Ci : 0.0) *
                                           ((bw && bw->xb_a) ? (bw->xb_out ? 3.0 : 2.0) : 1.0) +
                                       (double)g.Co * kred),
                     st);
#define IO_LAUNCH_NT_(TI_, TO_, BN_, STEM_, NBUF_, MINB_, BWE_, XF_, LIN_, XB_)                               \
    do {                                                                                                     \
        const size_t ldsz = (size_t)NBUF_ * (128 + BN_) * (BN_ == 64 ? 32 : 36) * sizeof(float);             \
        static std::atomic<unsigned long long> attr_done{0};                                                                       \
        if (io_first_on_device(attr_done)) {                                                                                    \
            (void)hipFuncSetAttribute(                                                                       \
                (const void*)conv_nt_kernel<TI_, TO_, BN_, STEM_, 4, NBUF_, MINB_, BWE_, XF_, LIN_, XB_>,    \
                hipFuncAttributeMaxDynamicSharedMemorySize, (int)ldsz);                                      \
        }                                                                                                    \
        hipLaunchKernelGGL((conv_nt_kernel<TI_, TO_, BN_, STEM_, 4, NBUF_, MINB_, BWE_, XF_, LIN_, XB_>),    \
                           grid, block, ldsz, st, g, (const TI_*)in, (const TI_*)wgt, (TO_*)out,             \
                           (const TO_*)add, (const TO_*)mask, ntn, in_bytes, w_bytes, out_bytes, st_mean,    \
                           st_m2, bws);                                                                      \
    } while (0)
#define IO_LAUNCH_NT__(TI_, TO_, BN_, STEM_, NBUF_, MINB_, LIN_)                                             \
    do {                                                                                                     \
        constexpr bool R_ = STEM_ == 0, XBOK_ = R_ && sizeof(TI_) == sizeof(TO_);                            \
        constexpr int XB1_ = XBOK_ ? 1 : 0, XB2_ = (XBOK_ && LIN_) ? 2 : XB1_;                               \
        constexpr int XB3_ = XB2_ == 2 ? 3 : XB1_;                                                           \
        if (XBOK_ && bws.xb_a && bws.xb_res == 2) IO_LAUNCH_NT_(TI_, TO_, BN_, STEM_, NBUF_, MINB_, false, false, LIN_, XB3_); \
        else if (XBOK_ && bws.xb_a && bws.xb_res) IO_LAUNCH_NT_(TI_, TO_, BN_, STEM_, NBUF_, MINB_, false, false, LIN_, XB2_); \
        else if (XBOK_ && bws.xb_a && bws.y) IO_LAUNCH_NT_(TI_, TO_, BN_, STEM_, NBUF_, MINB_, R_, false, LIN_, XB1_); \
        else if (XBOK_ && bws.xb_a) IO_LAUNCH_NT_(TI_, TO_, BN_, STEM_, NBUF_, MINB_, false, false, LIN_, XB1_);  \
        else if (R_ && bws.y) IO_LAUNCH_NT_(TI_, TO_, BN_, STEM_, NBUF_, MINB_, R_, false, LIN_, false);     \
        else if (R_ && bws.in_scale) IO_LAUNCH_NT_(TI_, TO_, BN_, STEM_, NBUF_, MINB_, false, R_, LIN_, false); \
        else IO_LAUNCH_NT_(TI_, TO_, BN_, STEM_, NBUF_, MINB_, false, false, LIN_, false);                   \
    } while (0)
#define IO_LAUNCH_NT(TI_, TO_, BN_, STEM_, NBUF_, MINB_)                                                     \
    do {                                                                                                     \
        if (STEM_ == 0 && lin) IO_LAUNCH_NT__(TI_, TO_, BN_, STEM_, NBUF_, MINB_, (STEM_ == 0));             \
        else IO_LAUNCH_NT__(TI_, TO_, BN_, STEM_, NBUF_, MINB_, false);                                      \
    } while (0)
    if (stem) {
        IO_REQUIRE(bn == 64, IO_ERR_SHAPE, "conv_nt(stem): Co must be 64");
        if (dt_in == IO_BF16) {
            IO_REQUIRE(dt_out == IO_BF16, IO_ERR_SHAPE, "conv_nt: bf16 operands write bf16 outputs");
            IO_LAUNCH_NT(bf16_t, bf16_t, 64, 1, 1, 4);
        } else if (dt_out == IO_BF16) {
            IO_LAUNCH_NT(float, bf16_t, 64, 1, 2, 1);
        } else if (g.cr && io_stem_rows_ok(g) && !add && !mask && !bws.y && !bws.in_scale) {
            return io_launch_stem_rows(g, (const float*)in, (const float*)wgt, (float*)out, st_mean, st_m2, bws.bias,
                                       bws.relu, st);
        } else if (g.cr) {
            IO_LAUNCH_NT(float, float, 64, 2, 1, 4);
        } else {
            IO_LAUNCH_NT(float, float, 64, 1, 2, 1);
        }
    } else if (dt_in == IO_BF16) {
        IO_REQUIRE(dt_out == IO_BF16, IO_ERR_SHAPE, "conv_nt: bf16 operands write bf16 outputs");
        if (bn == 128) IO_LAUNCH_NT(bf16_t, bf16_t, 128, 0, 1, 3);
        else IO_LAUNCH_NT(bf16_t, bf16_t, 64, 0, 1, 4);
    } else {
        IO_REQUIRE(dt_out == IO_F32, IO_ERR_SHAPE, "conv_nt: fp32 operands write fp32 outputs (except the stem)");
        if (bn == 128 && tiles > 768 && tiles <= 1024 && g.Th * g.Tw == 1) IO_LAUNCH_NT(float, float, 128, 0, 2, 1);
        else if (bn == 128) IO_LAUNCH_NT(float, float, 128, 0, 1, 3);
        else IO_LAUNCH_NT(float, float, 64, 0, 1, 4);
    }
#undef IO_LAUNCH_NT
#undef IO_LAUNCH_NT__
#undef IO_LAUNCH_NT_
    int rc = io_check_launch("conv_nt");
    if (rc || !bws.xb_bits) return rc;
    const size_t nwords = (size_t)M * g.Ci / 32;
    IO_REQUIRE(nwords / 256 + 1 < (1UL << 31), IO_ERR_SHAPE, "conv_nt: mask bits grid too large");
    const dim3 pgrid((unsigned)((nwords + 255) / 256));
    if (dt_in == IO_BF16)
        hipLaunchKernelGGL(pack_sign_bits_kernel<bf16_t>, pgrid, dim3(256), 0, st, (const bf16_t*)bws.xb_out, bws.xb_bits, nwords);
    else
        hipLaunchKernelGGL(pack_sign_bits_kernel<float>, pgrid, dim3(256), 0, st, (const float*)bws.xb_out, bws.xb_bits, nwords);
    return io_check_launch("conv_nt(mask bits)");
}

int io_launch_conv_wgrad(const IoConvGeom& g, const void* in, const void* dy, float* dw, float* partial,
                         size_t partial_bytes, int stem, hipStream_t st, int dt_in, int dt_dy) {
    IO_REQUIRE(g.Co % 64 == 0, IO_ERR_SHAPE, "conv_wgrad: Co=%d must be a multiple of 64", g.Co);
    IO_REQUIRE(!g.cr || (stem && dt_in == IO_F32 && g.cr > 0 && g.cr <= 8), IO_ERR_SHAPE,
               "conv_wgrad: the exact-K mode is for the fp32 stem (1..8 real channels)");
    if (stem)
        IO_REQUIRE(g.Ci == 8 && g.Co == 64 && (dt_in == IO_F32 || dt_dy == IO_BF16), IO_ERR_SHAPE,
                   "conv_wgrad(stem): need Ci=8, Co=64 (and bf16 dY with a bf16 input)");
    else
        IO_REQUIRE(g.Ci % 64 == 0 && dt_in == dt_dy, IO_ERR_SHAPE,
                   "conv_wgrad: Ci=%d must be a multiple of 64 (and one storage type)", g.Ci);
    IO_REQUIRE(g.N > 0 && g.Ho > 0 && g.Wo > 0 && g.Hi > 0 && g.Wi > 0, IO_ERR_SHAPE,
               "conv_wgrad: empty tensor (N=%d, in %dx%d, out %dx%d)", g.N, g.Hi, g.Wi, g.Ho, g.Wo);
    IO_REQUIRE(g.os == 1 && g.Ho == g.outH && g.Wo == g.outW, IO_ERR_SHAPE, "conv_wgrad: dY must be dense");
    IO_REQUIRE(!g.gw || (g.gw == 64 && !stem && g.Ci == g.Co), IO_ERR_SHAPE,
               "conv_wgrad: grouped mode needs a 64-channel window and Ci == Co");
    WgradPlan p = plan_wgrad(g, stem, dt_in == IO_F32 && dt_dy == IO_F32);
    const size_t need = io_conv_wgrad_partial_bytes(g, stem);
    IO_REQUIRE(partial_bytes >= need && (need == 0 || partial), IO_ERR_WORKSPACE,
               "conv_wgrad: workspace %zu < %zu bytes", partial_bytes, need);
    if (stem && dt_in == IO_F32 && dt_dy == IO_F32 && g.cr && io_stem_rows_ok(g))
        return io_launch_stem_wgrad_rows(g, (const float*)in, (const float*)dy, dw, partial, partial_bytes, st);
    if (stem && dt_in == IO_BF16 && dt_dy == IO_BF16) {
        const int rh = io_launch_stem_wgrad_halo(g, in, dy, dw, partial, partial_bytes, st, nullptr);
        if (rh <= 0) {
            g_last_wgrad_route.store(1, std::memory_order_relaxed);
            return rh;
        }
    }
    if (!stem && dt_in == IO_BF16 && dt_dy == IO_BF16) {
        const int rh = io_launch_conv_wgrad_halo3(g, in, dy, dw, partial, partial_bytes, st);
        if (rh <= 0) {
            g_last_wgrad_route.store(2, std::memory_order_relaxed);
            return rh;
        }
    }
    g_last_wgrad_route.store(0, std::memory_order_relaxed);
    if (dt_in == IO_F32 && dt_dy == IO_F32 && wgrad_wino_ok(g, stem)) {
        const WgradPlan pw = plan_wgrad_wino(g);
        float* dstw = pw.splits == 1 ? dw : partial;
        const size_t in_b = (size_t)4 * g.N * g.Hi * g.Wi * g.Ci, dy_b = (size_t)4 * g.N * g.Ho * g.Wo * g.Co;
        const double rows = (double)pw.kps * 64.0 + 64.0, samples = rows / ((double)g.Ho * g.Wo) + 2.0;
        IO_REQUIRE(rows * g.Co * 4.0 < 4.0e9 && samples * g.Hi * g.Wi * g.Ci * 4.0 < 4.0e9 && (double)g.N * g.Hi * g.Wi < 2.0e9,
                   IO_ERR_SHAPE, "conv_wgrad(wino): one split spans more than 4 GB (32-bit offsets)");
        const double Mdw = (double)g.N * g.Ho * g.Wo;
        IoProfScope prof(IO_PROF_WGRAD_WINO, 2.0 * Mdw * g.Co * 9.0 * g.Ci,
                         4.0 * (Mdw * g.Co + (double)g.N * g.Hi * g.Wi * g.Ci + 9.0 * g.Co * g.Ci), st,
                         2.0 * Mdw * g.Co * 9.0 * g.Ci * (g.Wo % 16 == 0 ? 0.5 : 2.0 / 3.0));
        if (g.Wo % 16 == 0) {
            hipLaunchKernelGGL(conv_wgrad_wino4_kernel, dim3((unsigned)(pw.tiles * pw.splits)), dim3(kThreads),
                               (size_t)2 * 6 * 64 * 16 * sizeof(float), st, g, (const float*)in, (const float*)dy, dstw,
                               pw.ntile_c, pw.tiles, pw.kps, in_b, dy_b);
        } else {
        const size_t lds = (size_t)2 * 4 * 64 * 36 * sizeof(float);
        static std::atomic<unsigned long long> attr_done{0};
        if (io_first_on_device(attr_done))
            (void)hipFuncSetAttribute((const void*)conv_wgrad_wino_kernel<2>, hipFuncAttributeMaxDynamicSharedMemorySize,
                                      (int)lds);
        hipLaunchKernelGGL((conv_wgrad_wino_kernel<2>), dim3((unsigned)(pw.tiles * pw.splits)), dim3(kThreads), lds, st, g,
                           (const float*)in, (const float*)dy, dstw, pw.ntile_c, pw.tiles, pw.kps, in_b, dy_b);
        }
        int rcw = io_check_launch("conv_wgrad(wino)");
        if (rcw) return rcw;
        if (pw.splits > 1) rcw = io_splitk_reduce(partial, dw, (size_t)g.Co * io_filter_row(g) / 4, pw.splits, st);
        return rcw;
    }
    float* dst = p.splits == 1 ? dw : partial;
    int splits = p.splits;
    dim3 grid((unsigned)(p.tiles * p.splits)), block(kThreads);
    const size_t in_bytes = (size_t)io_dtype_bytes(dt_in) * g.N * g.Hi * g.Wi * g.Ci;
    const size_t dy_bytes = (size_t)io_dtype_bytes(dt_dy) * g.N * g.Ho * g.Wo * g.Co;
    {
        const double rows = (double)p.kps * 32.0 + 64.0, samples = rows / ((double)g.Ho * g.Wo) + 2.0;
        IO_REQUIRE(rows * g.Co * io_dtype_bytes(dt_dy) < 4.0e9 &&
                       samples * g.Hi * g.Wi * g.Ci * io_dtype_bytes(dt_in) < 4.0e9 &&
                       (double)g.N * g.Hi * g.Wi < 2.0e9,
                   IO_ERR_SHAPE, "conv_wgrad: one split spans more than 4 GB (32-bit offsets)");
    }
    const double Md = (double)g.N * g.Ho * g.Wo;
    const double kred = stem ? (double)g.wT * 5.0 : (double)g.Th * g.Tw * (g.gw ? g.gw : g.Ci);
    const bool lin1x1 = g.Th * g.Tw == 1 && g.is == 1 && g.dh0 == 0 && g.dw0 == 0 && g.Hi == g.Ho && g.Wi == g.Wo;
// ... 122 lines not shown
```

### instaorder_amd/csrc/io_common.h

```cpp
#pragma once
#include <hip/hip_runtime.h>
#include <stdint.h>
#include <stddef.h>

#include "../../include/instaorder_hip.h"

void io_set_error(const char* fmt, ...);
int io_check_launch(const char* what);

#define IO_REQUIRE(cond, code, ...)        \
    do {                                   \
        if (!(cond)) {                     \
            io_set_error(__VA_ARGS__);     \
            return (code);                 \
        }                                  \
    } while (0)

static inline int io_cdiv(long a, long b) { return (int)((a + b - 1) / b); }

#include <atomic>
static inline int io_device_cu_count() {
    static std::atomic<int> cache[64];
    int dev = 0;
    if (hipGetDevice(&dev) != hipSuccess || dev < 0 || dev >= 64) return 256;
// ... 26 lines not shown
__device__ __forceinline__ float io_bf2f(bf16_t v) { return __builtin_bit_cast(float, (unsigned)v << 16); }
typedef __bf16 io_bf16x2 __attribute__((ext_vector_type(2)));
typedef float io_f32x2 __attribute__((ext_vector_type(2)));
__device__ __forceinline__ bf16_t io_f2bf(float f) { return __builtin_bit_cast(unsigned short, (__bf16)f); }
__device__ __forceinline__ unsigned io_f2bf2(float lo, float hi) {
    const io_f32x2 v = {lo, hi};
    return __builtin_bit_cast(unsigned, __builtin_convertvector(v, io_bf16x2));
}
__device__ __forceinline__ f32x4 io_ldv(const float* p) { return *reinterpret_cast<const f32x4*>(p); }
__device__ __forceinline__ f32x4 io_ldv(const bf16_t* p) {
    const uint2 r = *reinterpret_cast<const uint2*>(p);
    f32x4 v;
    v[0] = __builtin_bit_cast(float, r.x << 16);
    v[1] = __builtin_bit_cast(float, r.x & 0xffff0000u);
    v[2] = __builtin_bit_cast(float, r.y << 16);
    v[3] = __builtin_bit_cast(float, r.y & 0xffff0000u);
    return v;
}
__device__ __forceinline__ void io_stv(float* p, f32x4 v) { *reinterpret_cast<f32x4*>(p) = v; }
__device__ __forceinline__ void io_stv(bf16_t* p, f32x4 v) {
    uint2 r;
    r.x = io_f2bf2(v[0], v[1]);
    r.y = io_f2bf2(v[2], v[3]);
    *reinterpret_cast<uint2*>(p) = r;
}
#endif

struct IoFastDiv {
    unsigned magic;
    int shift;
};
static inline IoFastDiv io_fastdiv(int d) {
    IoFastDiv f;
    if (d <= 1) { f.magic = 0; f.shift = -1; return f; }
    int s = 0;
    while ((1LL << s) < d) ++s;
    const unsigned long long num = 1ULL << (31 + s);
    f.magic = (unsigned)((num + (unsigned long long)d - 1) / (unsigned long long)d);
    f.shift = s - 1;
    return f;
}

struct IoConvGeom {
    int N, Hi, Wi, Ci;
    int Ho, Wo, Co;
    int outH, outW;
    int os, ooh, oow;
    int is;
    int Th, Tw;
    int dh0, dhs, dw0, dws;
    int r0, rs, s0, ss;
    int S, wT;
    int gw;
    int cr;
    IoFastDiv fd_howo, fd_wo;
};
static inline int io_stem_kp(int wT, int cr) { return (wT * cr + 31) / 32 * 32; }
static inline void io_geom_finish(IoConvGeom& g) {
    g.fd_howo = io_fastdiv(g.Ho * g.Wo);
    g.fd_wo = io_fastdiv(g.Wo);
}

struct IoBwStats {
    const void* y;
    const float *mean, *rstd, *mscale, *mshift;
    float *p1, *p2;
    int Mg;
    void* a_out;
    const float* bias;
    int relu;
    const float *in_mean, *in_scale, *in_shift;
    int in_Mg;
    const void* xb_y;
    const float *xb_a, *xb_b, *xb_c;
    void* xb_out;
    int xb_Mg;
    int xb_res;
    uint32_t* xb_bits;
    float* wino_u;
    const uint32_t* maskbits;
};

bool io_wino_on();

int io_launch_conv_nt(const IoConvGeom& g, const void* in, const void* wgt, void* out, const void* add,
                      const void* mask, int stem, hipStream_t st, float* st_mean = nullptr,
                      float* st_m2 = nullptr, const IoBwStats* bw = nullptr, int dt_in = IO_F32,
                      int dt_out = IO_F32);
bool io_conv_p256_takes_xop(long M, int Ci, int Co, int Mg);
int io_launch_conv_p256(const IoConvGeom& g, const void* in, const void* wgt, void* out, const void* add, const void* mask,
                        hipStream_t st, float* st_mean, float* st_m2, const IoBwStats* bw, size_t in_bytes,
                        unsigned w_bytes, size_t out_bytes);
int io_bf16_persist_mode();
int io_launch_conv_halo3(const IoConvGeom& g, const void* in, const void* wgt, void* out, const void* add, const void* mask,
                         hipStream_t st, float* st_mean, float* st_m2, const IoBwStats* bw, size_t in_bytes,
                         unsigned w_bytes, size_t out_bytes);
int io_launch_conv_stem_halo(const IoConvGeom& g, const void* in, const void* wgt, void* out, hipStream_t st, float* st_mean,
                             float* st_m2, const IoBwStats* bw, size_t in_bytes, unsigned w_bytes, size_t out_bytes);
int io_bn_bwd_from_tiles(float* p1, float* p2, const void* dz, const void* y, int M, int C, int G,
                         const float* gamma, const float* mean, const float* rstd, float* dgamma, float* dbeta,
                         void* dy, float* coef, hipStream_t st, int dt = IO_F32);
int io_bn_bwd_coefs_from_tiles(float* p1, float* p2, int M, int C, int G, const float* gamma, const float* mean,
                               const float* rstd, float* dgamma, float* dbeta, float* coef, hipStream_t st);
int io_bn_bwd_coefs_t(const void* dz, const void* y, int M, int C, int G, const float* gamma, const float* mean,
                      const float* rstd, float* dgamma, float* dbeta, float* coef, float* partial,
                      size_t partial_floats, hipStream_t st, int dt, const float* mask_scale = nullptr,
                      const float* mask_shift = nullptr);
int io_bn_stats_finalize_t(const void* y, int M, int C, int G, const float* gamma, const float* beta,
                           float* running_mean, float* running_var, float momentum, float eps, float* mean,
                           float* rstd, float* scale, float* shift, float* partial, size_t partial_floats,
                           hipStream_t st, int dt);
int io_bn_apply_t(const void* y, int M, int C, int G, int per_group_tables, const float* mean, const float* scale,
                  const float* shift, const void* identity, const float* mean2, const float* scale2,
                  const float* shift2, int relu, void* out, hipStream_t st, int dt, uint32_t* bits = nullptr);
int io_bn_bwd_t(const void* dout, const void* act, const float* mask_scale, const float* mask_shift, const void* y,
                int M, int C, int G, const float* gamma, const float* mean, const float* rstd, float* dgamma,
                float* dbeta, void* dy, void* dz_out, float* partial, size_t partial_floats, float* coef,
                hipStream_t st, int dt);
int io_maxpool_fwd_t(const void* x, int N, int H, int W, int C, void* out, uint32_t* idx, hipStream_t st, int dt,
                     const float* xs = nullptr, const float* xh = nullptr, int G = 1, const float* xm = nullptr);
int io_maxpool_bwd_t(const void* dy, const uint32_t* idx, int N, int H, int W, int C, void* dx, hipStream_t st, int dt);
int io_avgpool_fc_fwd_t(const void* x, int N, int HW, int C, const float* w0, const float* b0, int K0,
                        const float* w1, const float* b1, int K1, float* pooled, float* logits, hipStream_t st,
                        int dt);
int io_avgpool_fc_bwd_t(const float* dlogits, const float* pooled, int N, int HW, int C, const float* w0, int K0,
                        const float* w1, int K1, const void* relu_mask, void* dx, float* dw0, float* db0, float* dw1,
                        float* db1, hipStream_t st, int dt);
int io_pack_planes_t(const float* const* planes, const long* sample_strides, int nplanes, int N, int H, int W,
                     void* out, hipStream_t st, int dt);
int io_filter_prepare_t(const float* w, int O, int T, int C, void* dst, int transpose, hipStream_t st, int dt);
int io_stem_pack_filter(const float* w, float* wp, int O, int T, int cr, hipStream_t st);
int io_stem_unpack_grad(const float* dwp, float* dw, int O, int T, int cr, hipStream_t st);
int io_bn_resid2_tables(const float* mean3, const float* scale3, const float* shift3, const float* meand,
                        const float* scaled, const float* shiftd, int G, int C, float* coef, hipStream_t st);
constexpr int kIoStatTileRows = 128;
int io_bn_finalize_tiles(float* tile_mean, float* tile_m2, int M, int C, int G, const float* gamma,
                         const float* beta, float* running_mean, float* running_var, float momentum, float eps,
                         float* mean, float* rstd, float* scale, float* shift, hipStream_t st);
int io_launch_conv_wgrad(const IoConvGeom& g, const void* in, const void* dy, float* dw, float* partial,
                         size_t partial_bytes, int stem, hipStream_t st, int dt_in = IO_F32, int dt_dy = IO_F32);
size_t io_conv_wgrad_partial_bytes(const IoConvGeom& g, int stem);

IoConvGeom io_geom_fwd(int N, int H, int W, int Cin, int Cout, int R, int S, int stride, int pad);
bool io_stem_rows_ok(const IoConvGeom& g);
int io_launch_stem_rows(const IoConvGeom& g, const float* x8, const float* wp, float* out, float* st_mean, float* st_m2,
                        const float* bias, int relu, hipStream_t st);
int io_stem_wgrad_rows_max_blocks();
struct IoStemXb {
    const float *y, *a, *b, *c, *mean, *scale, *shift;
    int G, tiles_per_group;
};
int io_launch_stem_wgrad_rows(const IoConvGeom& g, const float* x8, const float* dy, float* dwp, float* partial,
                              size_t partial_bytes, hipStream_t st, const IoStemXb* xb = nullptr);
size_t io_stem_wgrad_halo_partial_bytes();
bool io_stem_wgrad_halo_ok(const IoConvGeom& g, size_t partial_bytes, int G);
int io_launch_stem_wgrad_halo(const IoConvGeom& g, const void* x8, const void* dz, float* dw, float* partial, size_t partial_bytes,
                              hipStream_t st, const IoStemXb* xb);
size_t io_wgrad_halo3_partial_bytes();
bool io_wgrad_halo3_shape(const IoConvGeom& g);
int io_launch_conv_wgrad_halo3(const IoConvGeom& g, const void* x, const void* dy, float* dw, float* partial, size_t partial_bytes,
                               hipStream_t st);
int io_splitk_reduce(const float* partial, float* dst, size_t n4, int splits, hipStream_t st);
struct IoFilterTable {
    static constexpr int kMax = 64;
    int n;
    int start[kMax + 1];
// ... 23 lines not shown
```

### instaorder_amd/csrc/net.hip

```cpp
#include <stdio.h>
#include <string.h>

#include <vector>

#include "io_common.h"

namespace {

constexpr int kMaxGroups = 8;
constexpr float kBnEps = 1e-5f, kBnMomentum = 0.1f;

struct ConvL {
    int cin, cout, k, stride, pad, cin_store;
    long w_off;
};
struct BnL {
    int C;
    long g_off, b_off, run_off;
    int index;
};
struct Block {
    ConvL c1, c2, c3, cd;
    BnL b1, b2, b3, bd;
    bool down;
    int stride, inC, planes;
};

inline size_t align_up(size_t v, size_t a) { return (v + a - 1) / a * a; }

}

struct io_net {
    int dtype = IO_F32;
    int in_ch, n_heads, head_dims[2];
    ConvL stem;
    BnL bn1;
    std::vector<Block> blocks;
    long fcw_off[2], fcb_off[2];
    long param_floats, running_floats;
    int n_bn;
    long bn_channels;
    std::vector<io_tensor_info> tensors;
};

namespace {

void add_tensor(io_net* net, const char* name, int kind, int ndim, const long* shape, long numel_storage,
                int cin_storage, long* off_out, int bn_index = -1, long run_off = -1) {
    io_tensor_info t;
    memset(&t, 0, sizeof(t));
    snprintf(t.name, sizeof(t.name), "%s", name);
    t.kind = kind;
    t.ndim = ndim;
    for (int i = 0; i < ndim; ++i) t.shape[i] = shape[i];
    t.offset = net->param_floats;
    t.numel_storage = numel_storage;
    t.cin_storage = cin_storage;
    t.bn_index = bn_index;
    t.running_offset = run_off;
    *off_out = net->param_floats;
    net->param_floats = (long)align_up((size_t)(net->param_floats + numel_storage), 64);
    net->tensors.push_back(t);
}

ConvL add_conv(io_net* net, const char* name, int cout, int cin, int k, int stride, int pad) {
    ConvL c;
    c.cin = cin; c.cout = cout; c.k = k; c.stride = stride; c.pad = pad;
    c.cin_store = (cin % 32 == 0) ? cin : 8;
    char nm[64];
    snprintf(nm, sizeof(nm), "%s.weight", name);
    const long shape[4] = {cout, cin, k, k};
    add_tensor(net, nm, 0, 4, shape, (long)cout * k * k * c.cin_store, c.cin_store, &c.w_off);
    return c;
}

BnL add_bn(io_net* net, const char* name, int C) {
    BnL b;
    b.C = C;
    b.index = net->n_bn++;
    b.run_off = net->running_floats;
    net->running_floats += 2L * C;
    net->bn_channels += C;
    char nm[64];
    const long shape[1] = {C};
    snprintf(nm, sizeof(nm), "%s.weight", name);
    add_tensor(net, nm, 1, 1, shape, C, C, &b.g_off, b.index, b.run_off);
    snprintf(nm, sizeof(nm), "%s.bias", name);
    add_tensor(net, nm, 2, 1, shape, C, C, &b.b_off, b.index, b.run_off);
    return b;
}

constexpr size_t kNoBuf = ~(size_t)0;
struct BlockBufs {
    size_t y1, a1, y2, a2, y3, yd, out;
    size_t bits;
};
struct Plan {
    size_t y0, a0, p0, idx0, pooled;
    std::vector<BlockBufs> blk;
    size_t tables;
    size_t bn_partial, bn_partial_floats, coef;
    size_t tile_mean, tile_m2;
    size_t gbuf[5];
    size_t aside;
    size_t wt, wg_partial, wg_partial_bytes;
    size_t wop;
    size_t stem_wp, stem_dwp;
    size_t wt_all;
    size_t wfold, fbias;
    size_t wino_u;
    size_t total;
};

struct Arena {
    size_t top = 0;
    size_t take(size_t bytes) {
        const size_t o = top;
        top = align_up(top + bytes, 256);
        return o;
    }
};

Plan make_plan(const io_net* net, int N, int S, bool training, int SW = 0) {
    Plan p;
    Arena a;
    if (SW <= 0) SW = S;
    const int H0 = S / 2, H1 = S / 4, W0 = SW / 2;
    const size_t f = sizeof(float);
    const size_t e = (size_t)io_dtype_bytes(net->dtype);
    const size_t maxact = (size_t)N * H0 * W0 * 64 * e;
    p.wop = net->dtype == IO_BF16 ? a.take((size_t)net->param_floats * sizeof(bf16_t)) : 0;
    {
        const size_t sb = (size_t)64 * io_stem_kp(49, net->in_ch) * f;
        p.stem_wp = a.take(sb);
        p.stem_dwp = a.take(sb);
    }
    p.wfold = training ? 0 : a.take((size_t)net->param_floats * e);
    p.fbias = training ? 0 : a.take((size_t)net->bn_channels * f);
    p.wino_u = net->dtype == IO_F32 ? a.take((size_t)18 * 512 * 512 * f) : kNoBuf;
    p.tables = a.take((size_t)4 * kMaxGroups * net->bn_channels * f);
    p.bn_partial_floats = (size_t)3 * 1100 * 2048;
    p.bn_partial = a.take(p.bn_partial_floats * f);
    p.coef = a.take((size_t)3 * kMaxGroups * 2048 * f);
    p.pooled = a.take((size_t)N * 2048 * f);
    {
        const size_t tiles_x_c = (size_t)N * H0 * W0 * 64 / kIoStatTileRows + (size_t)kMaxGroups * 2048;
        const size_t fl = training ? tiles_x_c + tiles_x_c / 32 + (size_t)kMaxGroups * 2048 : 0;
        p.tile_mean = a.take(fl * f);
        p.tile_m2 = a.take(fl * f);
    }
    p.blk.resize(net->blocks.size());
    if (training) {
        p.y0 = a.take(maxact);
        p.a0 = kNoBuf;
        p.p0 = a.take((size_t)N * H1 * H1 * 64 * e);
        p.idx0 = a.take((size_t)N * H1 * H1 * 16 * sizeof(uint32_t));
        int H = H1;
        for (size_t i = 0; i < net->blocks.size(); ++i) {
            const Block& b = net->blocks[i];
            const int Ho = H / b.stride;
            BlockBufs& bb = p.blk[i];
            const long Mo = (long)N * Ho * Ho;
            const bool never = net->dtype == IO_F32 && Mo % kMaxGroups == 0 && (Mo / kMaxGroups) % kIoStatTileRows == 0;
            bb.y1 = a.take((size_t)N * H * H * b.planes * e);
            bb.a1 = (never && b.stride == 1) ? kNoBuf : a.take((size_t)N * H * H * b.planes * e);
            bb.y2 = a.take((size_t)N * Ho * Ho * b.planes * e);
            bb.a2 = never ? kNoBuf : a.take((size_t)N * Ho * Ho * b.planes * e);
            bb.y3 = a.take((size_t)N * Ho * Ho * b.planes * 4 * e);
            bb.yd = b.down ? a.take((size_t)N * Ho * Ho * b.planes * 4 * e) : 0;
            bb.out = a.take((size_t)N * Ho * Ho * b.planes * 4 * e);
            bb.bits = (net->dtype == IO_BF16 && Mo % 256 == 0) ? a.take((size_t)Mo * b.planes * 4 / 8) : kNoBuf;
            H = Ho;
        }
        for (int i = 0; i < 5; ++i) p.gbuf[i] = a.take(maxact);
        p.aside = net->dtype == IO_F32 ? a.take(maxact / 2) : kNoBuf;
        size_t wg = 0, wtmax = 0;
        {
            IoConvGeom g = io_geom_fwd(N, S, S, 8, 64, 7, 7, 2, 3);
            if (net->dtype == IO_F32) g.cr = net->in_ch;
            wg = io_conv_wgrad_partial_bytes(g, 1);
        }
        H = H1;
        for (const Block& b : net->blocks) {
            const ConvL* cs[4] = {&b.c1, &b.c2, &b.c3, b.down ? &b.cd : nullptr};
            for (int j = 0; j < 4; ++j) {
                if (!cs[j]) continue;
                const ConvL& c = *cs[j];
                const int Hin = (j == 2) ? H / b.stride : H;
                IoConvGeom g = io_geom_fwd(N, Hin, Hin, c.cin, c.cout, c.k, c.k, c.stride, c.pad);
                const size_t need = io_conv_wgrad_partial_bytes(g, 0);
                if (need > wg) wg = need;
                const size_t wsz = (size_t)c.cout * c.k * c.k * c.cin * e;
                if (wsz > wtmax) wtmax = wsz;
            }
            H /= b.stride;
        }
        p.wg_partial_bytes = wg;
        p.wg_partial = a.take(wg);
        p.wt = a.take(wtmax);
        p.wt_all = a.take((size_t)net->param_floats * e);
    } else {
        const size_t r0 = a.take(maxact), r1 = a.take(maxact), r2 = a.take(maxact), r3 = a.take(maxact),
                     r4 = a.take(maxact), r5 = a.take(maxact);
        p.y0 = r3; p.a0 = r1; p.p0 = r0; p.idx0 = 0;
        size_t xin = r0, xout = r5;
        for (size_t i = 0; i < net->blocks.size(); ++i) {
            BlockBufs& bb = p.blk[i];
            bb.y1 = r3; bb.a1 = r1; bb.y2 = r3; bb.a2 = r2; bb.y3 = r3; bb.yd = r4; bb.out = xout; bb.bits = kNoBuf;
            const size_t t = xin; xin = xout; xout = t;
        }
        for (int i = 0; i < 5; ++i) p.gbuf[i] = 0;
        p.aside = kNoBuf;
        p.wg_partial = p.wt = 0;
        p.wt_all = kNoBuf;
        p.wg_partial_bytes = 0;
    }
    p.total = a.top;
    return p;
}

struct FoldDesc {
    long w_off, g_off, b_off, run_off, bias_off;
    int rows, rowlen;
};
struct FoldTable {
    int n;
    FoldDesc d[56];
};
template <typename T>
__global__ __launch_bounds__(256) void fold_bn_kernel(FoldTable t, const float* __restrict__ params,
                                                     const float* __restrict__ running, float eps,
                                                     T* __restrict__ wout, float* __restrict__ bias) {
    const FoldDesc d = t.d[blockIdx.y];
    for (int row = blockIdx.x; row < d.rows; row += gridDim.x) {
        const float s = params[d.g_off + row] / sqrtf(running[d.run_off + d.rows + row] + eps);
        if (threadIdx.x == 0) bias[d.bias_off + row] = params[d.b_off + row] - running[d.run_off + row] * s;
        const float* src = params + d.w_off + (size_t)row * d.rowlen;
        T* dst = wout + d.w_off + (size_t)row * d.rowlen;
        for (int k = threadIdx.x; k < d.rowlen; k += 256) {
            if constexpr (sizeof(T) == 2) dst[k] = io_f2bf(src[k] * s);
            else dst[k] = src[k] * s;
        }
    }
}

#define IO_TRY(expr)            \
    do {                        \
        int rc_ = (expr);       \
        if (rc_) return rc_;    \
    } while (0)

struct Tables {
    float *mean, *rstd, *scale, *shift;
};

struct Ctx {
    const io_net* net;
    const float* params;
    float* running;
    float* grads;
    char* ws;
    Plan plan;
    int N, S, G;
    int SW;
    bool training;
    hipStream_t st;
    std::vector<long> chan_prefix;

    float* buf(size_t off) const { return reinterpret_cast<float*>(ws + off); }
    void* act(size_t off) const { return ws + off; }
    int dt() const { return net->dtype; }
    const void* wop(long w_off) const {
        return net->dtype == IO_BF16 ? (const void*)(reinterpret_cast<const bf16_t*>(ws + plan.wop) + w_off)
                                     : (const void*)(params + w_off);
    }
    const void* wfold(long w_off) const {
        return net->dtype == IO_BF16 ? (const void*)(reinterpret_cast<const bf16_t*>(ws + plan.wfold) + w_off)
                                     : (const void*)(reinterpret_cast<const float*>(ws + plan.wfold) + w_off);
    }
    float* fbias(const BnL& b) const { return buf(plan.fbias) + chan_prefix[b.index]; }
    Tables tables(const BnL& b) const {
        float* base = buf(plan.tables) + (size_t)4 * kMaxGroups * chan_prefix[b.index];
        const size_t gs = (size_t)kMaxGroups * b.C;
        return Tables{base, base + gs, base + 2 * gs, base + 3 * gs};
    }
};

bool stem_exact(const Ctx& c, const ConvL& L) { return L.cin_store == 8 && c.net->dtype == IO_F32; }

int conv_fwd(const Ctx& c, const ConvL& L, const void* x, void* y, int H, bool stats = false, const BnL* xf = nullptr,
             int Mout = 0, const BnL* xr = nullptr, const void* xr_id = nullptr, void* xr_out = nullptr,
             bool xr_two = false, uint32_t* xr_bits = nullptr) {
    IoConvGeom g = io_geom_fwd(c.N, H, H, L.cin_store, L.cout, L.k, L.k, L.stride, L.pad);
    const bool stem = L.cin_store == 8;
    const void* w = c.wop(L.w_off);
    if (stem_exact(c, L)) {
        g.cr = L.cin;
        IO_TRY(io_stem_pack_filter(c.params + L.w_off, c.buf(c.plan.stem_wp), L.cout, L.k * L.k, L.cin, c.st));
        w = c.buf(c.plan.stem_wp);
    }
    IoBwStats ep{};
    if (xf) {
        Tables t = c.tables(*xf);
        ep.in_mean = t.mean;
        ep.in_scale = t.scale;
        ep.in_shift = t.shift;
        ep.in_Mg = Mout / c.G;
    }
    const bool wino = c.plan.wino_u != kNoBuf && L.k == 3 && L.stride == 1 && c.dt() == IO_F32;
    if (wino) ep.wino_u = c.buf(c.plan.wino_u);
    if (xr) {
        Tables t = c.tables(*xr);
        ep.xb_y = xr_id;
        ep.xb_a = t.scale;
        ep.xb_b = t.mean;
        ep.xb_c = t.shift;
        ep.xb_out = xr_out;
        ep.xb_Mg = Mout / c.G;
        ep.xb_res = 1;
        ep.xb_bits = xr_bits;
        if (xr_two) {
            const size_t gs = (size_t)c.G * xr->C;
            ep.xb_a = c.buf(c.plan.coef);
            ep.xb_b = c.buf(c.plan.coef) + gs;
            ep.xb_c = c.buf(c.plan.coef) + 2 * gs;
            ep.xb_res = 2;
        }
    }
    return io_launch_conv_nt(g, x, w, y, nullptr, nullptr, stem, c.st,
                             stats ? c.buf(c.plan.tile_mean) : nullptr, stats ? c.buf(c.plan.tile_m2) : nullptr,
                             (xf || xr || wino) ? &ep : nullptr, c.dt(), c.dt());
}

int bn_prepare(const Ctx& c, const BnL& b, const void* y, int M, bool from_tiles = false) {
    Tables t = c.tables(b);
    if (c.training && from_tiles)
        return io_bn_finalize_tiles(c.buf(c.plan.tile_mean), c.buf(c.plan.tile_m2), M, b.C, c.G,
                                    c.params + b.g_off, c.params + b.b_off, c.running + b.run_off,
                                    c.running + b.run_off + b.C, kBnMomentum, kBnEps, t.mean, t.rstd, t.scale,
                                    t.shift, c.st);
    if (c.training)
        return io_bn_stats_finalize_t(y, M, b.C, c.G, c.params + b.g_off, c.params + b.b_off, c.running + b.run_off,
                                      c.running + b.run_off + b.C, kBnMomentum, kBnEps, t.mean, t.rstd, t.scale,
                                      t.shift, c.buf(c.plan.bn_partial), c.plan.bn_partial_floats, c.st, c.dt());
    return io_bn_eval_prepare(b.C, c.params + b.g_off, c.params + b.b_off, c.running + b.run_off,
                              c.running + b.run_off + b.C, kBnEps, t.mean, t.scale, t.shift, c.st);
}

int conv_bn(const Ctx& c, const ConvL& L, const BnL& b, const void* x, void* y, int Hin, int Mout,
            const BnL* xf = nullptr, const BnL* xr = nullptr, const void* xr_id = nullptr, void* xr_out = nullptr,
            bool xr_two = false, uint32_t* xr_bits = nullptr) {
    const bool fuse = c.training && (Mout / c.G) % kIoStatTileRows == 0;
    IO_TRY(conv_fwd(c, L, x, y, Hin, fuse, xf, Mout, xr, xr_id, xr_out, xr_two, xr_bits));
    return bn_prepare(c, b, y, Mout, fuse);
}

#ifndef IO_XB_BF16_MAXP
#define IO_XB_BF16_MAXP 64
#endif
#ifndef IO_XB_BF16_L1
#define IO_XB_BF16_L1 1
#endif
int out_rows(const Ctx& c, size_t i) {
    int H = c.S / 4;
    for (size_t k = 0; k <= i; ++k) H /= c.net->blocks[k].stride;
    return c.N * H * H;
}
int xr_route(const Ctx& c, size_t i) {
    if (!c.training || i + 1 >= c.net->blocks.size()) return 0;
    const Block& b = c.net->blocks[i];
    const int Mout = out_rows(c, i);
    if (Mout % c.G != 0 || (Mout / c.G) % kIoStatTileRows != 0) return 0;
    if (c.net->dtype == IO_F32) return 1;
    if (IO_XB_BF16_L1 && b.planes <= IO_XB_BF16_MAXP) return 1;
    return io_conv_p256_takes_xop(Mout, b.planes * 4, c.net->blocks[i + 1].planes, Mout / c.G) ? 2 : 0;
}

uint32_t* bits_of(const Ctx& c, size_t i) {
    const size_t off = c.plan.blk[i].bits;
    return (c.training && off != kNoBuf) ? reinterpret_cast<uint32_t*>(c.ws + off) : nullptr;
}

bool bits_written(const Ctx& c, size_t i) {
    return c.plan.blk[i].bits != kNoBuf && xr_route(c, i) != 1;
}

bool fuse_in(const Ctx& c, int Mout) {
    return c.training && c.net->dtype == IO_F32 && Mout % c.G == 0 && (Mout / c.G) % kIoStatTileRows == 0;
}

int bn_act(const Ctx& c, const BnL& b, const void* y, int M, const void* idt, const BnL* b2, int relu,
           void* out, uint32_t* bits = nullptr) {
    Tables t = c.tables(b);
    const float *m2 = nullptr, *s2 = nullptr, *h2 = nullptr;
    if (b2) {
        Tables t2 = c.tables(*b2);
        m2 = t2.mean;
        s2 = t2.scale;
        h2 = t2.shift;
    }
    return io_bn_apply_t(y, M, b.C, c.training ? c.G : 1, c.training ? 1 : 0, t.mean, t.scale, t.shift, idt, m2, s2,
                         h2, relu, out, c.st, c.dt(), bits);
}

int conv_folded(const Ctx& c, const ConvL& L, const BnL& b, const void* x, void* y, int H, int W, const void* add,
                int relu) {
    IoConvGeom g = io_geom_fwd(c.N, H, W, L.cin_store, L.cout, L.k, L.k, L.stride, L.pad);
    IoBwStats ep{};
    ep.bias = c.fbias(b);
    ep.relu = relu;
    if (c.plan.wino_u != kNoBuf && L.k == 3 && L.stride == 1 && c.dt() == IO_F32 && !add)
        ep.wino_u = c.buf(c.plan.wino_u);
    const void* w = c.wfold(L.w_off);
    if (stem_exact(c, L)) {
        g.cr = L.cin;
        IO_TRY(io_stem_pack_filter((const float*)w, c.buf(c.plan.stem_wp), L.cout, L.k * L.k, L.cin, c.st));
        w = c.buf(c.plan.stem_wp);
    }
    return io_launch_conv_nt(g, x, w, y, add, nullptr, L.cin_store == 8, c.st, nullptr, nullptr, &ep,
                             c.dt(), c.dt());
}

int run_forward_eval(Ctx& c, const void* x8, float* logits) {
    const io_net* net = c.net;
    const Plan& p = c.plan;
    const int H0 = c.S / 2, H1 = c.S / 4;
    {
        FoldTable t;
        t.n = 0;
        auto add = [&](const ConvL& L, const BnL& b) {
            FoldDesc& d = t.d[t.n++];
            d.w_off = L.w_off; d.g_off = b.g_off; d.b_off = b.b_off; d.run_off = b.run_off;
            d.bias_off = c.chan_prefix[b.index];
            d.rows = L.cout; d.rowlen = L.k * L.k * L.cin_store;
        };
        add(net->stem, net->bn1);
        for (const Block& b : net->blocks) {
            add(b.c1, b.b1); add(b.c2, b.b2); add(b.c3, b.b3);
            if (b.down) add(b.cd, b.bd);
        }
        IO_REQUIRE(t.n <= 56, IO_ERR_STATE, "fold table overflow");
        IoProfScope prof(IO_PROF_TRANSPOSE, 0.0, (4.0 + io_dtype_bytes(c.dt())) * (double)net->param_floats, c.st);
        if (c.dt() == IO_BF16)
            hipLaunchKernelGGL(fold_bn_kernel<bf16_t>, dim3(64, t.n), dim3(256), 0, c.st, t, c.params, c.running, kBnEps,
                               reinterpret_cast<bf16_t*>(c.ws + p.wfold), c.buf(p.fbias));
        else
            hipLaunchKernelGGL(fold_bn_kernel<float>, dim3(64, t.n), dim3(256), 0, c.st, t, c.params, c.running, kBnEps,
                               reinterpret_cast<float*>(c.ws + p.wfold), c.buf(p.fbias));
        IO_TRY(io_check_launch("fold_bn"));
    }
    const int W0 = c.SW / 2;
    IO_TRY(conv_folded(c, net->stem, net->bn1, x8, c.act(p.a0), c.S, c.SW, nullptr, 1));
    IO_TRY(io_maxpool_fwd_t(c.act(p.a0), c.N, H0, W0, 64, c.act(p.p0), nullptr, c.st, c.dt()));
    const void* x = c.act(p.p0);
    int H = H1, W = c.SW / 4;
    for (size_t i = 0; i < net->blocks.size(); ++i) {
        const Block& b = net->blocks[i];
        const BlockBufs& bb = p.blk[i];
        const int Ho = H / b.stride, Wo = W / b.stride;
        IO_TRY(conv_folded(c, b.c1, b.b1, x, c.act(bb.a1), H, W, nullptr, 1));
        IO_TRY(conv_folded(c, b.c2, b.b2, c.act(bb.a1), c.act(bb.a2), H, W, nullptr, 1));
        const void* identity = x;
        if (b.down) {
            IO_TRY(conv_folded(c, b.cd, b.bd, x, c.act(bb.yd), H, W, nullptr, 0));
            identity = c.act(bb.yd);
        }
        IO_TRY(conv_folded(c, b.c3, b.b3, c.act(bb.a2), c.act(bb.out), Ho, Wo, identity, 1));
        x = c.act(bb.out);
        H = Ho;
        W = Wo;
    }
    const float* w1 = net->n_heads > 1 ? c.params + net->fcw_off[1] : nullptr;
    const float* b1 = net->n_heads > 1 ? c.params + net->fcb_off[1] : nullptr;
    return io_avgpool_fc_fwd_t(x, c.N, H * W, 2048, c.params + net->fcw_off[0], c.params + net->fcb_off[0],
                               net->head_dims[0], w1, b1, net->n_heads > 1 ? net->head_dims[1] : 0, c.buf(p.pooled),
                               logits, c.st, c.dt());
}

int run_forward(Ctx& c, const void* x8, float* logits) {
    if (!c.training) return run_forward_eval(c, x8, logits);
    const io_net* net = c.net;
    const Plan& p = c.plan;
    const int H0 = c.S / 2, H1 = c.S / 4;
    if (c.dt() == IO_BF16)
        IO_TRY(io_filter_prepare_t(c.params, 1, 1, (int)net->param_floats, c.act(p.wop), 0, c.st, IO_BF16));
    IO_TRY(conv_bn(c, net->stem, net->bn1, x8, c.act(p.y0), c.S, c.N * H0 * H0));
    {
        Tables t = c.tables(net->bn1);
        IO_TRY(io_maxpool_fwd_t(c.act(p.y0), c.N, H0, H0, 64, c.act(p.p0), reinterpret_cast<uint32_t*>(c.ws + p.idx0),
                                c.st, c.dt(), t.scale, t.shift, c.G, t.mean));
    }
    const void* x = c.act(p.p0);
    int H = H1;
    const BnL* pend_bn = nullptr;
    const void *pend_y3 = nullptr, *pend_id = nullptr;
    bool pend_two = false;
    for (size_t i = 0; i < net->blocks.size(); ++i) {
        const Block& b = net->blocks[i];
        const BlockBufs& bb = p.blk[i];
        const int Ho = H / b.stride;
        const int Min = c.N * H * H, Mout = c.N * Ho * Ho;
        if (pend_bn) {
            IO_TRY(conv_bn(c, b.c1, b.b1, pend_y3, c.act(bb.y1), H, Min, nullptr, pend_bn, pend_id,
                           c.act(p.blk[i - 1].out), pend_two, xr_route(c, i - 1) == 2 ? bits_of(c, i - 1) : nullptr));
            pend_bn = nullptr;
        } else {
            IO_TRY(conv_bn(c, b.c1, b.b1, x, c.act(bb.y1), H, Min));
        }
        const bool f3 = fuse_in(c, Mout), f2 = f3 && b.stride == 1;
        IO_REQUIRE((f2 || bb.a1 != kNoBuf) && (f3 || bb.a2 != kNoBuf), IO_ERR_SHAPE,
                   "io_net_forward: G=%d does not divide this batch into whole 128-row tiles (use G in 1, 2, 4, 8)", c.G);
        if (f2) {
            IO_TRY(conv_bn(c, b.c2, b.b2, c.act(bb.y1), c.act(bb.y2), H, Mout, &b.b1));
        } else {
            IO_TRY(bn_act(c, b.b1, c.act(bb.y1), Min, nullptr, nullptr, 1, c.act(bb.a1)));
            IO_TRY(conv_bn(c, b.c2, b.b2, c.act(bb.a1), c.act(bb.y2), H, Mout));
        }
        if (f3) {
            IO_TRY(conv_bn(c, b.c3, b.b3, c.act(bb.y2), c.act(bb.y3), Ho, Mout, &b.b2));
        } else {
            IO_TRY(bn_act(c, b.b2, c.act(bb.y2), Mout, nullptr, nullptr, 1, c.act(bb.a2)));
            IO_TRY(conv_bn(c, b.c3, b.b3, c.act(bb.a2), c.act(bb.y3), Ho, Mout));
        }
        if (b.down) {
            IO_TRY(conv_bn(c, b.cd, b.bd, x, c.act(bb.yd), H, Mout));
            if (xr_route(c, i)) {
                Tables t3 = c.tables(b.b3), td = c.tables(b.bd);
                IO_TRY(io_bn_resid2_tables(t3.mean, t3.scale, t3.shift, td.mean, td.scale, td.shift, c.G, b.b3.C,
                                           c.buf(c.plan.coef), c.st));
                pend_bn = &b.b3;
                pend_y3 = c.act(bb.y3);
                pend_id = c.act(bb.yd);
                pend_two = true;
            } else {
                IO_TRY(bn_act(c, b.b3, c.act(bb.y3), Mout, c.act(bb.yd), &b.bd, 1, c.act(bb.out), bits_of(c, i)));
            }
        } else if (xr_route(c, i)) {
            pend_bn = &b.b3;
            pend_y3 = c.act(bb.y3);
            pend_id = x;
            pend_two = false;
        } else {
            IO_TRY(bn_act(c, b.b3, c.act(bb.y3), Mout, x, nullptr, 1, c.act(bb.out), bits_of(c, i)));
        }
        x = c.act(bb.out);
        H = Ho;
    }
    const float* w1 = net->n_heads > 1 ? c.params + net->fcw_off[1] : nullptr;
    const float* b1 = net->n_heads > 1 ? c.params + net->fcb_off[1] : nullptr;
    IO_TRY(io_avgpool_fc_fwd_t(x, c.N, H * H, 2048, c.params + net->fcw_off[0], c.params + net->fcb_off[0],
                               net->head_dims[0], w1, b1, net->n_heads > 1 ? net->head_dims[1] : 0, c.buf(p.pooled),
                               logits, c.st, c.dt()));
    return IO_OK;
}

int bn_back(const Ctx& c, const BnL& b, const void* dout, int mask, const void* act, const void* y, int M,
            void* dy, void* dz_out) {
    Tables t = c.tables(b);
    return io_bn_bwd_t(dout, mask == 2 ? act : nullptr, mask == 1 ? t.scale : nullptr, mask == 1 ? t.shift : nullptr,
                       y, M, b.C, c.G, c.params + b.g_off, t.mean, t.rstd, c.grads + b.g_off, c.grads + b.b_off, dy,
                       dz_out, c.buf(c.plan.bn_partial), c.plan.bn_partial_floats, c.buf(c.plan.coef), c.st, c.dt());
}

int conv_wgrad(const Ctx& c, const ConvL& L, const void* x, const void* dy, int H) {
    IoConvGeom g = io_geom_fwd(c.N, H, H, L.cin_store, L.cout, L.k, L.k, L.stride, L.pad);
    const bool stem = L.cin_store == 8;
    if (stem_exact(c, L)) {
        g.cr = L.cin;
        IO_TRY(io_launch_conv_wgrad(g, x, dy, c.buf(c.plan.stem_dwp), c.buf(c.plan.wg_partial), c.plan.wg_partial_bytes,
                                    1, c.st, c.dt(), c.dt()));
        return io_stem_unpack_grad(c.buf(c.plan.stem_dwp), c.grads + L.w_off, L.cout, L.k * L.k, L.cin, c.st);
    }
    return io_launch_conv_wgrad(g, x, dy, c.grads + L.w_off, c.buf(c.plan.wg_partial), c.plan.wg_partial_bytes, stem,
                                c.st, c.dt(), c.dt());
}

int transpose_filters(const Ctx& c) {
    if (c.plan.wt_all == kNoBuf) return IO_OK;
    IoFilterTable tab;
    tab.n = 0;
    tab.start[0] = 0;
    for (const Block& b : c.net->blocks) {
        const ConvL* cs[4] = {&b.c1, &b.c2, &b.c3, b.down ? &b.cd : nullptr};
        for (int j = 0; j < 4; ++j)
            if (cs[j]) IO_TRY(io_filter_table_add(tab, cs[j]->w_off, cs[j]->cout, cs[j]->k * cs[j]->k, cs[j]->cin));
    }
    return io_filter_transpose_all(tab, c.params, c.act(c.plan.wt_all), c.st, c.dt());
// ... 278 lines not shown
            b.c3 = add_conv(net, nm, b.planes * 4, b.planes, 1, 1, 0);
            snprintf(nm, sizeof(nm), "layer%d.%d.bn3", li + 1, bi);
            b.b3 = add_bn(net, nm, b.planes * 4);
            if (b.down) {
                snprintf(nm, sizeof(nm), "layer%d.%d.downsample.0", li + 1, bi);
                b.cd = add_conv(net, nm, b.planes * 4, inC, 1, b.stride, 0);
                snprintf(nm, sizeof(nm), "layer%d.%d.downsample.1", li + 1, bi);
                b.bd = add_bn(net, nm, b.planes * 4);
            }
            inC = b.planes * 4;
            net->blocks.push_back(b);
        }
    const char* hn1[1] = {"fc"};
    const char* hn2[2] = {"fc_occ", "fc_depth"};
    for (int i = 0; i < n_heads; ++i) {
        char nm[64];
        const char* base = n_heads == 1 ? hn1[0] : hn2[i];
        const long ws[2] = {head_dims[i], 2048};
        snprintf(nm, sizeof(nm), "%s.weight", base);
        add_tensor(net, nm, 3, 2, ws, (long)head_dims[i] * 2048, 2048, &net->fcw_off[i]);
        const long bs[1] = {head_dims[i]};
        snprintf(nm, sizeof(nm), "%s.bias", base);
        add_tensor(net, nm, 4, 1, bs, head_dims[i], head_dims[i], &net->fcb_off[i]);
    }
    return net;
}

extern "C" void io_net_destroy(io_net* net) { delete net; }
extern "C" int io_net_set_dtype(io_net* net, int dtype) {
    IO_REQUIRE(dtype == IO_F32 || dtype == IO_BF16, IO_ERR_SHAPE, "io_net_set_dtype: unknown dtype %d", dtype);
    net->dtype = dtype;
    return IO_OK;
}
extern "C" int io_net_get_dtype(const io_net* net) { return net->dtype; }
extern "C" long io_net_param_floats(const io_net* net) { return net->param_floats; }
extern "C" long io_net_running_floats(const io_net* net) { return net->running_floats; }
extern "C" int io_net_num_tensors(const io_net* net) { return (int)net->tensors.size(); }
extern "C" int io_net_num_logits(const io_net* net) { return net->head_dims[0] + net->head_dims[1]; }

extern "C" int io_net_tensor_info(const io_net* net, int i, io_tensor_info* out) {
    IO_REQUIRE(i >= 0 && i < (int)net->tensors.size(), IO_ERR_SHAPE, "tensor index %d out of range", i);
    *out = net->tensors[i];
    return IO_OK;
}

static int check_shape(int N, int S, int G) {
    IO_REQUIRE(S >= 32 && S % 32 == 0, IO_ERR_SHAPE, "input size S=%d must be a multiple of 32", S);
    IO_REQUIRE(N >= 1 && G >= 1 && G <= kMaxGroups && N % G == 0, IO_ERR_SHAPE, "N=%d G=%d (G<=%d, G | N)", N, G,
               kMaxGroups);
    IO_REQUIRE((double)N * S * S < 2.0e9, IO_ERR_SHAPE, "N=%d x S=%d: more than 2^31 input pixels", N, S);
    return IO_OK;
}

extern "C" size_t io_net_workspace_bytes(const io_net* net, int N, int S, int training) {
    if (check_shape(N, S, 1)) return 0;
    return make_plan(net, N, S, training != 0).total;
}

extern "C" long io_net_activation_offset(const io_net* net, int N, int S, int which) {
    if (check_shape(N, S, 1)) return -1;
    const Plan p = make_plan(net, N, S, true);
    const int nb = (int)net->blocks.size();
    if (which == 0) return (long)p.y0;
    if (which == 1) {
        io_set_error("io_net_activation_offset: relu(bn1(.)) is not stored (it is evaluated inside the pooling kernel)");
        return -1;
    }
    if (which == 2) return (long)p.p0;
    if (which >= 3 && which < 3 + nb) return (long)p.blk[which - 3].out;
    io_set_error("io_net_activation_offset: which=%d (0..%d)", which, 2 + nb);
    return -1;
}

static void fill_ctx(Ctx& c, io_net* net, const float* params, float* running, float* grads, int N, int S, int G,
                     bool training, void* ws, hipStream_t st, int SW = 0) {
    c.net = net;
    c.params = params;
    c.running = running;
    c.grads = grads;
    c.ws = (char*)ws;
    c.N = N; c.S = S; c.G = G;
    c.SW = SW > 0 ? SW : S;
    c.training = training;
    c.st = st;
    c.plan = make_plan(net, N, S, training, c.SW);
    c.chan_prefix.assign(net->n_bn, 0);
    std::vector<int> Cs(net->n_bn, 0);
    Cs[net->bn1.index] = net->bn1.C;
    for (const Block& b : net->blocks) {
        Cs[b.b1.index] = b.b1.C;
        Cs[b.b2.index] = b.b2.C;
        Cs[b.b3.index] = b.b3.C;
        if (b.down) Cs[b.bd.index] = b.bd.C;
    }
    long acc = 0;
    for (int i = 0; i < net->n_bn; ++i) { c.chan_prefix[i] = acc; acc += Cs[i]; }
}

extern "C" int io_net_forward(io_net* net, const float* params, float* running, const void* x8, int N, int S,
                              int G, int training, void* ws, size_t ws_bytes, float* logits, hipStream_t st) {
    IO_TRY(check_shape(N, S, G));
    IO_REQUIRE(training || G == 1, IO_ERR_SHAPE, "eval forward uses running statistics: G must be 1");
    Ctx c;
    fill_ctx(c, net, params, running, nullptr, N, S, G, training != 0, ws, st);
    IO_REQUIRE(ws_bytes >= c.plan.total, IO_ERR_WORKSPACE, "io_net_forward: workspace %zu < %zu bytes", ws_bytes,
               c.plan.total);
    return run_forward(c, x8, logits);
}

static int check_shape_hw(int N, int H, int W) {
    IO_REQUIRE(H >= 32 && H % 32 == 0 && W >= 32 && W % 32 == 0, IO_ERR_SHAPE,
               "input %d x %d: both sides must be multiples of 32 (five stride-2 stages)", H, W);
    IO_REQUIRE(N >= 1 && (double)N * H * W < 2.0e9, IO_ERR_SHAPE, "N=%d x %d x %d: more than 2^31 input pixels", N, H, W);
    return IO_OK;
}
extern "C" size_t io_net_workspace_bytes_hw(const io_net* net, int N, int H, int W) {
    if (check_shape_hw(N, H, W)) return 0;
    return make_plan(net, N, H, false, W).total;
}
extern "C" int io_net_forward_eval_hw(io_net* net, const float* params, float* running, const void* x8, int N, int H,
                                      int W, void* ws, size_t ws_bytes, float* logits, hipStream_t st) {
    IO_TRY(check_shape_hw(N, H, W));
    Ctx c;
    fill_ctx(c, net, params, running, nullptr, N, H, 1, false, ws, st, W);
    IO_REQUIRE(ws_bytes >= c.plan.total, IO_ERR_WORKSPACE, "io_net_forward_eval_hw: workspace %zu < %zu bytes", ws_bytes,
               c.plan.total);
    return run_forward_eval(c, x8, logits);
}

extern "C" int io_net_backward(io_net* net, const float* params, float* grads, const void* x8,
                               const float* dlogits, int N, int S, int G, void* ws, size_t ws_bytes,
                               hipStream_t st) {
    IO_TRY(check_shape(N, S, G));
    Ctx c;
    fill_ctx(c, net, params, nullptr, grads, N, S, G, true, ws, st);
    IO_REQUIRE(ws_bytes >= c.plan.total, IO_ERR_WORKSPACE, "io_net_backward: workspace %zu < %zu bytes", ws_bytes,
               c.plan.total);
    return run_backward(c, dlogits, x8);
}

extern "C" int io_net_backward_stages(io_net* net, const float* params, float* grads, const void* x8,
                                      const float* dlogits, int N, int S, int G, void* ws, size_t ws_bytes,
                                      int stage_lo, int stage_hi, hipStream_t st) {
    IO_TRY(check_shape(N, S, G));
    IO_REQUIRE(stage_lo >= 0 && stage_lo < stage_hi && stage_hi <= kBwdStages, IO_ERR_SHAPE,
               "io_net_backward_stages: stages [%d, %d) outside [0, %d)", stage_lo, stage_hi, kBwdStages);
    Ctx c;
    fill_ctx(c, net, params, nullptr, grads, N, S, G, true, ws, st);
    IO_REQUIRE(ws_bytes >= c.plan.total, IO_ERR_WORKSPACE, "io_net_backward_stages: workspace %zu < %zu bytes", ws_bytes,
               c.plan.total);
    return run_backward(c, dlogits, x8, stage_lo, stage_hi);
}

extern "C" int io_net_backward_num_stages(const io_net*) { return kBwdStages; }
```

Baseline: 1821 pairs/s.

## Pack ReLU masks as bits inside conv epilogue and read bitmasks in backward

Removes the separate pack_sign_bits kernel by building the residual ReLU sign bitmask inside the conv_nt epilogue, using DPP lane exchanges and byte permutes to assemble 32-bit words. The bitmask is now also enabled for fp32 and controlled by a new IO_NT_MASKBITS toggle that defaults to on. Backward epilogues read one bit per element from it instead of a full fp32/bf16 mask tensor, which cuts mask-read traffic and saves a kernel launch. The cost is added epilogue work and cross-lane shuffles, plus the risk that the intricate bit-placement logic is wrong.

```diff
diff --git a/include/instaorder_hip.h b/include/instaorder_hip.h
--- a/include/instaorder_hip.h
+++ b/include/instaorder_hip.h
@@ -288,6 +288,8 @@
                            float* tile_mean, float* tile_m2, int dtype, hipStream_t stream);
 int io_set_bf16_p256_xop(int on);
 int io_get_bf16_p256_xop(void);
+int io_set_nt_maskbits(int on);
+int io_get_nt_maskbits(void);
 typedef struct io_weight_desc {
     long src, dst_op, dst_t, dst_g;
     int Co, Ci, T, Cop, Cip;
diff --git a/instaorder_amd/_lib.py b/instaorder_amd/_lib.py
--- a/instaorder_amd/_lib.py
+++ b/instaorder_amd/_lib.py
@@ -65,6 +65,8 @@
     "io_set_bf16_p256": (_I, [_I]),
     "io_get_bf16_p256": (_I, []),
     "io_set_bf16_p256_xop": (_I, [_I]),
+    "io_set_nt_maskbits": (_I, [_I]),
+    "io_get_nt_maskbits": (_I, []),
     "io_get_bf16_p256_xop": (_I, []),
     "io_conv2d_fwd_resid_dt": (_I, [_P, _P, _P, _P, _P, _P, _I, _I, _I, _I, _I, _I, _I, _P, _P, _P, _P, _P, _I, _P]),
     "io_debug_last_nt_route": (_I, []),
diff --git a/instaorder_amd/csrc/capi.hip b/instaorder_amd/csrc/capi.hip
--- a/instaorder_amd/csrc/capi.hip
+++ b/instaorder_amd/csrc/capi.hip
@@ -39,6 +39,22 @@
 extern "C" int io_set_winograd(int on) {
     const int prev = io_wino_on() ? 1 : 0;
     g_wino.store(on ? 1 : 0, std::memory_order_relaxed);
+    return prev;
+}
+static std::atomic<int> g_nt_maskbits{-1};
+bool io_nt_maskbits_on() {
+    int v = g_nt_maskbits.load(std::memory_order_relaxed);
+    if (v < 0) {
+        const char* e = getenv("IO_NT_MASKBITS");
+        v = (e && e[0] == '0') ? 0 : 1;
+        g_nt_maskbits.store(v, std::memory_order_relaxed);
+    }
+    return v != 0;
+}
+extern "C" int io_get_nt_maskbits(void) { return io_nt_maskbits_on() ? 1 : 0; }
+extern "C" int io_set_nt_maskbits(int on) {
+    const int prev = io_nt_maskbits_on() ? 1 : 0;
+    g_nt_maskbits.store(on ? 1 : 0, std::memory_order_relaxed);
     return prev;
 }
 extern "C" const char* io_last_error_string(void) { return g_err; }
diff --git a/instaorder_amd/csrc/conv_igemm.hip b/instaorder_amd/csrc/conv_igemm.hip
--- a/instaorder_amd/csrc/conv_igemm.hip
+++ b/instaorder_amd/csrc/conv_igemm.hip
@@ -77,6 +77,13 @@
 }
 template <> __device__ __forceinline__ void st_el_s<bf16_t>(float v, __amdgpu_buffer_rsrc_t r, unsigned off, unsigned soff) {
     __builtin_amdgcn_raw_buffer_store_b16(io_f2bf(v), r, off, soff, kStAux);
+}
+template <typename T> __device__ __forceinline__ unsigned ld_raw(__amdgpu_buffer_rsrc_t r, unsigned off, unsigned soff = 0);
+template <> __device__ __forceinline__ unsigned ld_raw<float>(__amdgpu_buffer_rsrc_t r, unsigned off, unsigned soff) {
+    return __builtin_amdgcn_raw_buffer_load_b32(r, off, soff, 0);
+}
+template <> __device__ __forceinline__ unsigned ld_raw<bf16_t>(__amdgpu_buffer_rsrc_t r, unsigned off, unsigned soff) {
+    return (unsigned)(unsigned short)__builtin_amdgcn_raw_buffer_load_b16(r, off, soff, 0);
 }
 typedef __bf16 bf16x8 __attribute__((ext_vector_type(8)));
 
@@ -206,6 +213,10 @@
     const __amdgpu_buffer_rsrc_t rs_y = make_rsrc_at(XB ? bw.xb_y : (const void*)in, xb_base, XB ? in_bytes : xb_base);
     const __amdgpu_buffer_rsrc_t rs_side =
         make_rsrc_at((XB && bw.xb_out) ? bw.xb_out : (void*)out, xb_base, (XB && bw.xb_out && n0 == 0) ? in_bytes : xb_base);
+    constexpr bool XBITS = LIN && XB >= 2;
+    const __amdgpu_buffer_rsrc_t rs_xbits =
+        make_rsrc_at((XBITS && bw.xb_bits) ? (void*)bw.xb_bits : (void*)out, xb_base / (8 * ES),
+                     (XBITS && bw.xb_bits && n0 == 0) ? in_bytes / (8 * ES) : xb_base / (8 * ES));
     int th = 0, tw = 0, cc = 0;
     const float rcr = 1.0f / (float)(XK ? g.cr : 1), rS = 1.0f / (float)g.S;
     auto load_tile = [&](int kt) {
@@ -444,6 +455,44 @@
 #pragma unroll
                 for (int j = 0; j < AR; ++j)
                     __builtin_amdgcn_raw_buffer_store_b128(__builtin_bit_cast(u32x4, ra[j]), rs_side, rowv[j], xaoff, 0);
+                if constexpr (XBITS) {
+                    static_assert(AR == 4, "four rows per thread");
+                    unsigned p = 0;
+#pragma unroll
+                    for (int j = 0; j < AR; ++j) {
+                        if constexpr (ES == 4) {
+#pragma unroll
+                            for (int e = 0; e < 4; ++e) p |= (ra[j][e] > 0.f ? 1u : 0u) << (8 * j + e);
+                        } else {
+                            const u32x4 raw = __builtin_bit_cast(u32x4, ra[j]);
+#pragma unroll
+                            for (int d = 0; d < 4; ++d) {
+                                p |= (__builtin_bit_cast(float, raw[d] << 16) > 0.f ? 1u : 0u) << (8 * j + 2 * d);
+                                p |= (__builtin_bit_cast(float, raw[d] & 0xffff0000u) > 0.f ? 1u : 0u) << (8 * j + 2 * d + 1);
+                            }
+                        }
+                    }
+                    constexpr int X1 = 0xB1, X2 = 0x4E, HM = 0x141;
+                    const auto xchg = [](unsigned v, auto ctrl) {
+                        return (unsigned)__builtin_amdgcn_update_dpp(0, (int)v, decltype(ctrl)::value, 0xF, 0xF, true);
+                    };
+                    if constexpr (ES == 4) {
+                        p <<= (unsigned)(kq & 1) * 4u;
+                        p |= xchg(p, std::integral_constant<int, X1>{});
+                    }
+                    const int up1 = ES == 4 ? (kq >> 1) & 1 : kq & 1;
+                    const int hb = ES == 4 ? ((kq >> 1) ^ (kq >> 2)) & 1 : kq & 1;
+                    const unsigned sel1 = (0x05010400u ^ (up1 ? 0x04040404u : 0u)) + (hb ? 0x02020202u : 0u);
+                    const unsigned q = ES == 4 ? xchg(p, std::integral_constant<int, X2>{}) : xchg(p, std::integral_constant<int, X1>{});
+                    p = __builtin_amdgcn_perm(q, p, sel1);
+                    const int up2 = ES == 4 ? (kq >> 2) & 1 : (kq >> 1) & 1;
+                    const unsigned r = ES == 4 ? xchg(p, std::integral_constant<int, HM>{}) : xchg(p, std::integral_constant<int, X2>{});
+                    p = __builtin_amdgcn_perm(r, p, up2 ? 0x03020706u : 0x05040100u);
+                    const int jrow = 2 * hb + up2;
+                    const unsigned rv = jrow == 0 ? rowv[0] : jrow == 1 ? rowv[1] : jrow == 2 ? rowv[2] : rowv[3];
+                    const unsigned boff = ((rv + xaoff) >> (ES == 4 ? 5 : 4)) & ~3u;
+                    __builtin_amdgcn_raw_buffer_store_b32(p, rs_xbits, (ES == 2 || (kq & 1) == 0) ? boff : kInvalidOff, 0, 0);
+                }
             } else {
 #pragma unroll
                 for (int j = 0; j < AR; ++j)
@@ -648,6 +697,17 @@
     const __amdgpu_buffer_rsrc_t rs_add = make_rsrc_at(add ? (const void*)add : (const void*)out, out_base, out_bytes);
     const __amdgpu_buffer_rsrc_t rs_mask = make_rsrc_at(mask ? (const void*)mask : (const void*)out, out_base, out_bytes);
     const __amdgpu_buffer_rsrc_t rs_bwy = make_rsrc_at(bw.y ? bw.y : (const void*)out, out_base, out_bytes);
+    const bool mbit = bw.maskbits != nullptr;
+    constexpr int MSH = OS == 4 ? 5 : 4;
+    constexpr unsigned MLO = (unsigned)OS - 1u;
+    const __amdgpu_buffer_rsrc_t rs_mbits = make_rsrc_at(mbit ? (const void*)bw.maskbits : (const void*)out, out_base / (8 * OS),
+                                                         mbit ? out_bytes / (8 * OS) : out_base / (8 * OS));
+    const __amdgpu_buffer_rsrc_t rs_maskx = mbit ? rs_mbits : rs_mask;
+    const unsigned mbitpos = (unsigned)lane & (8u * OS - 1u);
+    auto mask_off = [&](unsigned off) { return mbit ? ((off >> MSH) & ~MLO) : off; };
+    auto mask_keep = [&](unsigned raw) {
+        return mbit ? ((raw >> mbitpos) & 1u) != 0u : __builtin_bit_cast(float, raw << (32 - 8 * OS)) > 0.f;
+    };
     float bw_mu[TJ], bw_rs[TJ], bw_sc[TJ], bw_sh[TJ], bw_s1[TJ], bw_s2[TJ];
     if constexpr (BWE) {
         const int gcol = (m0 / bw.Mg) * g.Co + n0 + wn * (BN / WN) + (lane & 31);
@@ -664,8 +724,9 @@
         const unsigned rowstep = (unsigned)g.Co * (unsigned)OS;
         const unsigned lane_base = (unsigned)(m0 - opix_lo + wm * 64 + RQ * 4 * (lane >> 5)) * rowstep + colb2;
         const __amdgpu_buffer_rsrc_t rs_add0 = add ? rs_add : make_rsrc(out, 0);
-        const __amdgpu_buffer_rsrc_t rs_mask0 = mask ? rs_mask : make_rsrc(out, 0);
-        const bool nomask = mask == nullptr;
+        const __amdgpu_buffer_rsrc_t rs_mask0 = (mask || mbit) ? rs_maskx : make_rsrc(out, 0);
+        const bool nomask = mask == nullptr && !mbit;
+        const unsigned mrowstep = mbit ? rowstep >> MSH : rowstep;
         const __amdgpu_buffer_rsrc_t rs_aout = make_rsrc_at(bw.a_out ? bw.a_out : (void*)out, out_base,
                                                             bw.a_out ? out_bytes : out_base);
         constexpr bool ROWS = OS == 2 && BN == 128;
@@ -677,17 +738,19 @@
 #pragma unroll
             for (int j = 0; j < TJ; ++j) {
                 const unsigned voff = lane_base + (unsigned)(i * RI) * rowstep + (unsigned)j * 32u * OS;
-                float av[16], mv[16], yv[16];
+                float av[16], yv[16];
+                unsigned mv[16];
+                const unsigned mvoff = mask_off(voff);
 #pragma unroll
                 for (int r = 0; r < 16; ++r) yv[r] = ld_el_s<TO>(rs_bwy, voff, (unsigned)(RQ * ((r & 3) + 8 * (r >> 2))) * rowstep);
 #pragma unroll
                 for (int r = 0; r < 16; ++r) av[r] = ld_el_s<TO>(rs_add0, voff, (unsigned)(RQ * ((r & 3) + 8 * (r >> 2))) * rowstep);
 #pragma unroll
-                for (int r = 0; r < 16; ++r) mv[r] = ld_el_s<TO>(rs_mask0, voff, (unsigned)(RQ * ((r & 3) + 8 * (r >> 2))) * rowstep);
+                for (int r = 0; r < 16; ++r) mv[r] = ld_raw<TO>(rs_mask0, mvoff, (unsigned)(RQ * ((r & 3) + 8 * (r >> 2))) * mrowstep);
 #pragma unroll
                 for (int r = 0; r < 16; ++r) {
                     float v = acc[i][j][r] + av[r];
-                    v = (mv[r] > 0.f || nomask) ? v : 0.f;
+                    v = (mask_keep(mv[r]) || nomask) ? v : 0.f;
                     const float t = __builtin_fmaf(yv[r] - bw_mu[j], bw_sc[j], bw_sh[j]);
                     if (bw.mscale) v = t > 0.f ? v : 0.f;
                     bw_s1[j] += v;
@@ -719,7 +782,7 @@
         const unsigned rowstep = (unsigned)g.Co * (unsigned)OS;
         const unsigned lane_base = (unsigned)((wm * 64 + 4 * (lane >> 5)) * g.Co + n0 + wn * (BN / WN) + (lane & 31)) * (unsigned)OS;
         if constexpr (OS == 2 && BN == 128) {
-            if (!add && !mask) {
+            if (!add && !mask && !mbit) {
                 constexpr int WC = BN / WN, EPP = WC + 4, LPR = WC / 4, RPI = 64 / LPR, NI = 32 / RPI;
                 __syncthreads();
                 float* ep = smem + wave * (32 * EPP);
@@ -768,12 +831,13 @@
                         acc[i][j][r] = (bw.relu && v < 0.f) ? 0.f : v;
                     }
                 }
-                if (mask) {
-                    float mv[16];
-#pragma unroll
-                    for (int r = 0; r < 16; ++r) mv[r] = ld_el_s<TO>(rs_mask, voff, (unsigned)((r & 3) + 8 * (r >> 2)) * rowstep);
-#pragma unroll
-                    for (int r = 0; r < 16; ++r) acc[i][j][r] = mv[r] > 0.f ? acc[i][j][r] : 0.f;
+                if (mask || mbit) {
+                    unsigned mv[16];
+                    const unsigned mvoff = mask_off(voff), mrowstep = mbit ? rowstep >> MSH : rowstep;
+#pragma unroll
+                    for (int r = 0; r < 16; ++r) mv[r] = ld_raw<TO>(rs_maskx, mvoff, (unsigned)((r & 3) + 8 * (r >> 2)) * mrowstep);
+#pragma unroll
+                    for (int r = 0; r < 16; ++r) acc[i][j][r] = mask_keep(mv[r]) ? acc[i][j][r] : 0.f;
                 }
 #pragma unroll
                 for (int r = 0; r < 16; ++r) {
@@ -820,15 +884,15 @@
                     acc[i][j][r] = (bw.relu && v < 0.f) ? 0.f : v;
                 }
         }
-        if (mask) {
+        if (mask || mbit) {
 #pragma unroll
             for (int j = 0; j < TJ; ++j) {
-                float mv[16];
+                unsigned mv[16];
 #pragma unroll
                 for (int r = 0; r < 16; ++r)
-                    mv[r] = ld_el<TO>(rs_mask, rowb[r] == kInvalidOff ? kInvalidOff : rowb[r] + j * JS);
-#pragma unroll
-                for (int r = 0; r < 16; ++r) acc[i][j][r] = mv[r] > 0.f ? acc[i][j][r] : 0.f;
+                    mv[r] = ld_raw<TO>(rs_maskx, rowb[r] == kInvalidOff ? kInvalidOff : mask_off(rowb[r] + j * JS));
+#pragma unroll
+                for (int r = 0; r < 16; ++r) acc[i][j][r] = mask_keep(mv[r]) ? acc[i][j][r] : 0.f;
             }
         }
 #pragma unroll
@@ -2442,22 +2506,6 @@
         for (int k = 1; k < 8; ++k) s += red[k][tx];
         reinterpret_cast<f32x4*>(dst)[i] = s;
     }
-}
-
-template <typename T>
-__global__ __launch_bounds__(256) void pack_sign_bits_kernel(const T* __restrict__ t, uint32_t* __restrict__ bits,
-                                                             size_t nwords) {
-    const size_t i = (size_t)blockIdx.x * 256 + threadIdx.x;
-    if (i >= nwords) return;
-    const T* p = t + i * 32;
-    uint32_t w = 0;
-#pragma unroll
-    for (int q = 0; q < 8; ++q) {
-        const f32x4 v = io_ldv(p + 4 * q);
-#pragma unroll
-        for (int e = 0; e < 4; ++e) w |= (v[e] > 0.f ? 1u : 0u) << (4 * q + e);
-    }
-    bits[i] = w;
 }
 
 inline size_t io_filter_row(const IoConvGeom& g) {
@@ -2620,6 +2668,9 @@
     g_last_route.store(0, std::memory_order_relaxed);
     IO_REQUIRE(!bws.xb_bits || (bws.xb_res && bws.xb_out), IO_ERR_SHAPE,
                "conv_nt: xb_bits is the mask of the residual forms' side output (needs xb_res and xb_out)");
+    IO_REQUIRE(!bws.maskbits || (mask && g.Co % 32 == 0), IO_ERR_SHAPE,
+               "conv_nt: maskbits goes with mask (the same mask, one bit per element), 32 | Co");
+    const void* const kmask = bws.maskbits ? nullptr : mask;
     static std::atomic<int> small_tiles_c{-1};
     int small_tiles = small_tiles_c.load(std::memory_order_relaxed);
     if (small_tiles < 0) {
@@ -2703,7 +2754,8 @@
     const double kred = stem ? (double)g.wT * 5.0 : (double)g.Th * g.Tw * (g.gw ? g.gw : g.Ci);
     IoProfScope prof(stem ? IO_PROF_CONV_STEM : (bn == 128 ? IO_PROF_CONV_NT128 : IO_PROF_CONV_NT64),
                      2.0 * (double)M * g.Co * kred,
-                     (double)os * M * g.Co * (1.0 + (add ? 1.0 : 0.0) + (mask ? 1.0 : 0.0) + ((bw && bw->y) ? 1.0 : 0.0)) +
+                     (double)os * M * g.Co * (1.0 + (add ? 1.0 : 0.0) + (kmask ? 1.0 : 0.0) + ((bw && bw->y) ? 1.0 : 0.0)) +
+                         (bws.maskbits ? (double)M * g.Co / 8.0 : 0.0) + (bws.xb_bits ? (double)M * g.Ci / 8.0 : 0.0) +
                          (double)es * ((kred > 0.0 ? (double)g.N * g.Hi * g.Wi * g.Ci : 0.0) *
                                            ((bw && bw->xb_a) ? (bw->xb_out ? 3.0 : 2.0) : 1.0) +
                                        (double)g.Co * kred),
@@ -2719,7 +2771,7 @@
         }                                                                                                    \
         hipLaunchKernelGGL((conv_nt_kernel<TI_, TO_, BN_, STEM_, 4, NBUF_, MINB_, BWE_, XF_, LIN_, XB_>),    \
                            grid, block, ldsz, st, g, (const TI_*)in, (const TI_*)wgt, (TO_*)out,             \
-                           (const TO_*)add, (const TO_*)mask, ntn, in_bytes, w_bytes, out_bytes, st_mean,    \
+                           (const TO_*)add, (const TO_*)kmask, ntn, in_bytes, w_bytes, out_bytes, st_mean,   \
                            st_m2, bws);                                                                      \
     } while (0)
 #define IO_LAUNCH_NT__(TI_, TO_, BN_, STEM_, NBUF_, MINB_, LIN_)                                             \
@@ -2768,16 +2820,7 @@
 #undef IO_LAUNCH_NT
 #undef IO_LAUNCH_NT__
 #undef IO_LAUNCH_NT_
-    int rc = io_check_launch("conv_nt");
-    if (rc || !bws.xb_bits) return rc;
-    const size_t nwords = (size_t)M * g.Ci / 32;
-    IO_REQUIRE(nwords / 256 + 1 < (1UL << 31), IO_ERR_SHAPE, "conv_nt: mask bits grid too large");
-    const dim3 pgrid((unsigned)((nwords + 255) / 256));
-    if (dt_in == IO_BF16)
-        hipLaunchKernelGGL(pack_sign_bits_kernel<bf16_t>, pgrid, dim3(256), 0, st, (const bf16_t*)bws.xb_out, bws.xb_bits, nwords);
-    else
-        hipLaunchKernelGGL(pack_sign_bits_kernel<float>, pgrid, dim3(256), 0, st, (const float*)bws.xb_out, bws.xb_bits, nwords);
-    return io_check_launch("conv_nt(mask bits)");
+    return io_check_launch("conv_nt");
 }
 
 int io_launch_conv_wgrad(const IoConvGeom& g, const void* in, const void* dy, float* dw, float* partial,
diff --git a/instaorder_amd/csrc/io_common.h b/instaorder_amd/csrc/io_common.h
--- a/instaorder_amd/csrc/io_common.h
+++ b/instaorder_amd/csrc/io_common.h
@@ -132,6 +132,7 @@
 };
 
 bool io_wino_on();
+bool io_nt_maskbits_on();
 
 int io_launch_conv_nt(const IoConvGeom& g, const void* in, const void* wgt, void* out, const void* add,
                       const void* mask, int stem, hipStream_t st, float* st_mean = nullptr,
diff --git a/instaorder_amd/csrc/net.hip b/instaorder_amd/csrc/net.hip
--- a/instaorder_amd/csrc/net.hip
+++ b/instaorder_amd/csrc/net.hip
@@ -41,6 +41,7 @@
     int n_bn;
     long bn_channels;
     std::vector<io_tensor_info> tensors;
+    int fwd_nt_bits = -1;
 };
 
 namespace {
@@ -169,7 +170,8 @@
             bb.y3 = a.take((size_t)N * Ho * Ho * b.planes * 4 * e);
             bb.yd = b.down ? a.take((size_t)N * Ho * Ho * b.planes * 4 * e) : 0;
             bb.out = a.take((size_t)N * Ho * Ho * b.planes * 4 * e);
-            bb.bits = (net->dtype == IO_BF16 && Mo % 256 == 0) ? a.take((size_t)Mo * b.planes * 4 / 8) : kNoBuf;
+            bb.bits = (net->dtype == IO_BF16 ? Mo % 256 == 0 : (b.planes * 4) % 32 == 0) ? a.take((size_t)Mo * b.planes * 4 / 8)
+                                                                                         : kNoBuf;
             H = Ho;
         }
         for (int i = 0; i < 5; ++i) p.gbuf[i] = a.take(maxact);
@@ -264,6 +266,7 @@
     int N, S, G;
     int SW;
     bool training;
+    bool nt_bits;
     hipStream_t st;
     std::vector<long> chan_prefix;
 
@@ -378,11 +381,12 @@
 
 uint32_t* bits_of(const Ctx& c, size_t i) {
     const size_t off = c.plan.blk[i].bits;
-    return (c.training && off != kNoBuf) ? reinterpret_cast<uint32_t*>(c.ws + off) : nullptr;
+    if (!c.training || off == kNoBuf || (c.net->dtype == IO_F32 && !c.nt_bits)) return nullptr;
+    return reinterpret_cast<uint32_t*>(c.ws + off);
 }
 
 bool bits_written(const Ctx& c, size_t i) {
-    return c.plan.blk[i].bits != kNoBuf && xr_route(c, i) != 1;
+    return bits_of(c, i) != nullptr && (xr_route(c, i) != 1 || c.nt_bits);
 }
 
 bool fuse_in(const Ctx& c, int Mout) {
@@ -502,7 +506,7 @@
         const int Min = c.N * H * H, Mout = c.N * Ho * Ho;
         if (pend_bn) {
             IO_TRY(conv_bn(c, b.c1, b.b1, pend_y3, c.act(bb.y1), H, Min, nullptr, pend_bn, pend_id,
-                           c.act(p.blk[i - 1].out), pend_two, xr_route(c, i - 1) == 2 ? bits_of(c, i - 1) : nullptr));
+                           c.act(p.blk[i - 1].out), pend_two, bits_written(c, i - 1) ? bits_of(c, i - 1) : nullptr));
             pend_bn = nullptr;
         } else {
             IO_TRY(conv_bn(c, b.c1, b.b1, x, c.act(bb.y1), H, Min));
@@ -947,6 +951,7 @@
     c.N = N; c.S = S; c.G = G;
     c.SW = SW > 0 ? SW : S;
     c.training = training;
+    c.nt_bits = io_nt_maskbits_on();
     c.st = st;
     c.plan = make_plan(net, N, S, training, c.SW);
     c.chan_prefix.assign(net->n_bn, 0);
@@ -970,6 +975,7 @@
     fill_ctx(c, net, params, running, nullptr, N, S, G, training != 0, ws, st);
     IO_REQUIRE(ws_bytes >= c.plan.total, IO_ERR_WORKSPACE, "io_net_forward: workspace %zu < %zu bytes", ws_bytes,
                c.plan.total);
+    if (training) net->fwd_nt_bits = c.nt_bits ? 1 : 0;
     return run_forward(c, x8, logits);
 }
 
@@ -1001,6 +1007,7 @@
     fill_ctx(c, net, params, nullptr, grads, N, S, G, true, ws, st);
     IO_REQUIRE(ws_bytes >= c.plan.total, IO_ERR_WORKSPACE, "io_net_backward: workspace %zu < %zu bytes", ws_bytes,
                c.plan.total);
+    if (net->fwd_nt_bits >= 0) c.nt_bits = net->fwd_nt_bits != 0;
     return run_backward(c, dlogits, x8);
 }
 
@@ -1014,6 +1021,7 @@
     fill_ctx(c, net, params, nullptr, grads, N, S, G, true, ws, st);
     IO_REQUIRE(ws_bytes >= c.plan.total, IO_ERR_WORKSPACE, "io_net_backward_stages: workspace %zu < %zu bytes", ws_bytes,
                c.plan.total);
+    if (net->fwd_nt_bits >= 0) c.nt_bits = net->fwd_nt_bits != 0;
     return run_backward(c, dlogits, x8, stage_lo, stage_hi);
 }
 
```

Result: no change. 1835 pairs/s (median of 6 runs) (+0.8%).
